# borgwang/tinynn-autograd

Hardware: NVIDIA B200
Metric: MLP train samples/sec (higher is better)
Workload: dtype f32 (tensor-core GEMMs: 3-term split on scaled fp16 hi/lo planes, fp32 accumulate)

## Files before the change

core/_backend.py:

```python
import ctypes
import gc
import os
import weakref

import numpy as np

_HERE = os.path.dirname(os.path.abspath(__file__))
_ROOT = os.path.dirname(_HERE)
LIB_PATH = os.environ.get(
    "TNN_B200_LIB", os.path.join(_ROOT, "tinynn-autograd_b200", "libtnn_b200.so"))

F32 = np.dtype(np.float32)
F64 = np.dtype(np.float64)
_DT_CODE = {F32: 0, F64: 1}
MAX_DIMS = 8

ADD, SUB, MUL, DIV, POW, MAXIMUM, MINIMUM, GE, GT, LE, LT, EQ = range(12)
MUL_GE, MUL_GT, MUL_LE, MUL_LT, MUL_EQ, DIV_BWD_B, POW_BWD_A, POW_BWD_B = range(20, 28)
NEG, EXP, LOG, COPY, CLIP, SCALE, CLIP_BWD, RECIP_MUL = range(40, 48)
RED_SUM, RED_MAX, RED_MIN = 0, 1, 2
OPT_SGD, OPT_ADAM, OPT_RMSPROP, OPT_MOMENTUM, OPT_ADAGRAD, OPT_ADADELTA = range(6)

_c_i64 = ctypes.c_int64
_c_i32 = ctypes.c_int32
_c_int = ctypes.c_int
_c_vp = ctypes.c_void_p
_c_dbl = ctypes.c_double
_c_sz = ctypes.c_size_t

_lib = None
_inited = False


class BackendError(RuntimeError):
    pass


_SIGNATURES = {
    "tnn_init": [_c_int],
    "tnn_shutdown": [],
    "tnn_sync": [],
    "tnn_device_info": [_c_vp, _c_vp, _c_vp, _c_vp, _c_vp],
    "tnn_device_count": [_c_vp],
    "tnn_alloc": [_c_sz, _c_vp],
    "tnn_free": [_c_vp],
    "tnn_pool_stats": [_c_vp, _c_vp, _c_vp],
    "tnn_pool_trim": [],
    "tnn_h2d": [_c_vp, _c_vp, _c_sz],
    "tnn_d2h": [_c_vp, _c_vp, _c_sz],
    "tnn_d2d": [_c_vp, _c_vp, _c_sz],
    "tnn_memset": [_c_vp, _c_int, _c_sz],
    "tnn_host_alloc": [_c_sz, _c_vp],
    "tnn_host_free": [_c_vp],
    "tnn_host_register": [_c_vp, _c_sz],
    "tnn_host_unregister": [_c_vp],
    "tnn_h2d_async_copy_stream": [_c_vp, _c_vp, _c_sz],
    "tnn_copy_stream_sync": [],
    "tnn_copy_wait_compute": [],
    "tnn_compute_wait_copy": [],
    "tnn_event_create": [_c_vp],
    "tnn_event_destroy": [_c_vp],
    "tnn_event_record": [_c_vp],
    "tnn_event_elapsed_ms": [_c_vp, _c_vp, _c_vp],
    "tnn_prof_enable": [_c_int],
    "tnn_prof_collect": [_c_vp, _c_vp],
    "tnn_l2_flush": [],
    "tnn_graph_begin": [],
    "tnn_graph_end": [_c_vp],
    "tnn_graph_abort": [],
    "tnn_graph_launch": [_c_vp],
    "tnn_graph_info": [_c_vp, _c_vp, _c_vp, _c_vp],
    "tnn_graph_destroy": [_c_vp],
    "tnn_ew": [_c_int, _c_int, _c_vp, _c_vp, _c_vp, _c_vp, _c_int, _c_vp, _c_vp, _c_vp, _c_vp,
               _c_dbl, _c_dbl, _c_int],
    "tnn_ew_flat": [_c_int, _c_int, _c_vp, _c_vp, _c_vp, _c_vp, _c_i64, _c_int, _c_dbl, _c_dbl,
                    _c_int],
    "tnn_cast": [_c_int, _c_vp, _c_int, _c_vp, _c_i64],
    "tnn_fill": [_c_int, _c_vp, _c_dbl, _c_i64],
    "tnn_reduce": [_c_int, _c_int, _c_vp, _c_vp, _c_i64, _c_i64, _c_i64],
    "tnn_unbroadcast": [_c_int, _c_vp, _c_vp, _c_int, _c_vp, _c_vp],
    "tnn_strided_copy": [_c_int, _c_vp, _c_vp, _c_int, _c_vp, _c_vp, _c_vp],
    "tnn_gather_rows": [_c_int, _c_vp, _c_vp, _c_vp, _c_i64, _c_i64, _c_i64],
    "tnn_scatter_rows": [_c_int, _c_vp, _c_vp, _c_vp, _c_i64, _c_i64, _c_i64],
    "tnn_gather_flat": [_c_int, _c_vp, _c_vp, _c_vp, _c_i64],
    "tnn_scatter_flat": [_c_int, _c_vp, _c_vp, _c_vp, _c_i64],
    "tnn_gemm_simt": [_c_int, _c_vp, _c_i64, _c_vp, _c_i64, _c_i64, _c_vp, _c_i64, _c_i64, _c_i64,
                      _c_i64, _c_i64, _c_vp, _c_int, _c_vp, _c_vp],
    "tnn_dense_bwd_simt": [_c_int, _c_vp, _c_vp, _c_vp, _c_vp, _c_vp, _c_vp, _c_vp, _c_int, _c_vp, _c_int,
                           _c_i64, _c_i64, _c_i64],
    "tnn_split_tf32": [_c_vp, _c_i64, _c_i64, _c_vp, _c_vp, _c_i64, _c_vp, _c_vp, _c_i64],
    "tnn_gemm_tf32x3": [_c_vp, _c_i64, _c_vp, _c_vp, _c_i64, _c_vp, _c_vp, _c_i64, _c_i64, _c_i64,
                        _c_i64, _c_vp, _c_int, _c_int, _c_vp, _c_vp, _c_vp, _c_i64, _c_vp],
    "tnn_split_tf32_bf16": [_c_vp, _c_i64, _c_i64, _c_vp, _c_vp, _c_vp, _c_i64],
    "tnn_gemm_tf32_bf16x2": [_c_vp, _c_i64, _c_vp, _c_vp, _c_vp, _c_i64, _c_vp, _c_vp, _c_vp, _c_i64,
                             _c_i64, _c_i64, _c_i64, _c_vp, _c_int, _c_int, _c_vp, _c_vp, _c_vp, _c_vp,
                             _c_i64, _c_vp],
    "tnn_f16_stats": [_c_vp, _c_i64, _c_vp, _c_int],
    "tnn_set_gemm_f16_cluster": [_c_int],
    "tnn_f16_meta_reset": [_c_vp],
    "tnn_split_f16": [_c_vp, _c_i64, _c_i64, _c_vp, _c_vp, _c_i64, _c_vp, _c_int],
    "tnn_gemm_f16x3": [_c_vp, _c_i64, _c_vp, _c_vp, _c_i64, _c_vp, _c_vp, _c_vp, _c_i64, _c_vp, _c_i64,
                       _c_i64, _c_i64, _c_vp, _c_int, _c_int, _c_vp, _c_vp, _c_vp],
    "tnn_split_tf32_bf16_cond": [_c_vp, _c_i64, _c_i64, _c_vp, _c_vp, _c_vp, _c_i64, _c_int,
                                 _c_vp, _c_i64, _c_i64, _c_vp, _c_vp, _c_vp, _c_i64, _c_int, _c_vp, _c_vp, _c_vp],
    "tnn_f16_stats_cond": [_c_vp, _c_i64, _c_vp, _c_int],
    "tnn_gemm_tf32_bf16x2_cond": [_c_vp, _c_i64, _c_vp, _c_vp, _c_vp, _c_i64, _c_vp, _c_vp, _c_vp, _c_i64,
                                  _c_i64, _c_i64, _c_i64, _c_vp, _c_int, _c_int, _c_vp, _c_vp, _c_vp, _c_vp],
    "tnn_set_gemm_cta_group": [_c_int],
    "tnn_set_gemm_ksplit": [_c_int],
    "tnn_set_gemm_group_m": [_c_int],
    "tnn_relu_fwd": [_c_int, _c_vp, _c_vp, _c_i64],
    "tnn_relu_bwd": [_c_int, _c_vp, _c_vp, _c_vp, _c_i64],
    "tnn_colsum": [_c_int, _c_vp, _c_vp, _c_i64, _c_i64],
    "tnn_ce_stats": [_c_int, _c_vp, _c_i64, _c_i64, _c_vp],
    "tnn_ce_merge_stats": [_c_int, _c_vp, _c_vp, _c_int],
    "tnn_ce_loss": [_c_int, _c_vp, _c_int, _c_vp, _c_i64, _c_i64, _c_vp, _c_dbl, _c_vp, _c_vp, _c_vp],
    "tnn_ce_fwd_small": [_c_int, _c_vp, _c_int, _c_vp, _c_i64, _c_i64, _c_dbl, _c_vp, _c_vp, _c_vp, _c_vp],
    "tnn_ce_bwd": [_c_int, _c_vp, _c_vp, _c_int, _c_vp, _c_i64, _c_i64, _c_vp, _c_vp, _c_dbl, _c_vp, _c_vp,
                   _c_vp],
    "tnn_set_gemm_reserved_sms": [_c_int],
    "tnn_d2h_async": [_c_vp, _c_vp, _c_sz, _c_vp],
    "tnn_event_sync": [_c_vp],
    "tnn_one_hot": [_c_int, _c_vp, _c_vp, _c_i64, _c_i64],
    "tnn_mlp_tail_workspace": [_c_int, _c_vp, _c_vp, _c_i64, _c_vp, _c_vp, _c_vp],
    "tnn_mlp_tail_step": [_c_int, _c_vp, _c_vp, _c_vp, _c_vp, _c_vp, _c_vp, _c_i64, _c_vp, _c_vp, _c_int,
                          _c_i64, _c_dbl, _c_vp, _c_vp, _c_vp, _c_vp, _c_vp, _c_vp, _c_vp],
    "tnn_opt_step": [_c_int, _c_int, _c_vp, _c_vp, _c_vp, _c_vp, _c_vp, _c_i64, _c_vp, _c_int],
    "tnn_opt_step_dev": [_c_int, _c_int, _c_vp, _c_vp, _c_vp, _c_vp, _c_vp, _c_i64, _c_vp],
    "tnn_nccl_unique_id": [_c_vp],
    "tnn_nccl_init": [_c_int, _c_int, _c_vp],
    "tnn_nccl_destroy": [],
    "tnn_allreduce_sum": [_c_int, _c_vp, _c_i64],
    "tnn_allgather": [_c_int, _c_vp, _c_vp, _c_i64],
    "tnn_comm_wait_compute": [],
    "tnn_compute_wait_comm": [],
    "tnn_allreduce_sum_comm": [_c_int, _c_vp, _c_i64],
    "tnn_nccl_version": [_c_vp],
}
EXPORTED_SYMBOLS = sorted(list(_SIGNATURES) + ["tnn_last_error", "tnn_stream", "tnn_launch_count",
                                                "tnn_alloc_ptr"])


def load_library():
    global _lib
    if _lib is not None:
        return _lib
    if not os.path.exists(LIB_PATH):
        raise BackendError(
            "libtnn_b200.so not found at %s -- build it with `python tinynn-autograd_b200/build.py` "
            "(there is no CPU fallback)" % LIB_PATH)
    lib = ctypes.CDLL(LIB_PATH)
    for name, argtypes in _SIGNATURES.items():
        fn = getattr(lib, name)
        fn.argtypes = argtypes
        fn.restype = _c_int
    lib.tnn_last_error.argtypes = []
    lib.tnn_last_error.restype = ctypes.c_char_p
    lib.tnn_stream.argtypes = []
    lib.tnn_stream.restype = _c_vp
    lib.tnn_launch_count.argtypes = []
    lib.tnn_launch_count.restype = ctypes.c_uint64
    lib.tnn_alloc_ptr.argtypes = [_c_sz]
    lib.tnn_alloc_ptr.restype = _c_vp
    _lib = lib
    return lib


def _raise(name):
    msg = _lib.tnn_last_error().decode("utf-8", "replace")
    raise BackendError("%s failed: %s" % (name, msg))


def init(device=None):
    global _inited
    if _inited:
        return
    lib = load_library()
    if device is None:
        device = int(os.environ.get("TNN_DEVICE", os.environ.get("LOCAL_RANK", "0")))
    if lib.tnn_init(int(device)):
        _raise("tnn_init")
    _inited = True


def is_initialized():
    return _inited


def sync():
    init()
    if _lib.tnn_sync():
        _raise("tnn_sync")


def launch_count():
    return int(_lib.tnn_launch_count()) if _lib is not None else 0


def device_info():
    init()
    sm, maj, mnr = _c_int(), _c_int(), _c_int()
    tot, l2 = _c_sz(), _c_sz()
    if _lib.tnn_device_info(ctypes.byref(sm), ctypes.byref(maj), ctypes.byref(mnr),
                            ctypes.byref(tot), ctypes.byref(l2)):
        _raise("tnn_device_info")
    return {"sm_count": sm.value, "cc": (maj.value, mnr.value), "total_mem": tot.value,
            "l2_bytes": l2.value}


def set_gemm_reserved_sms(n):
    init()
    if _lib.tnn_set_gemm_reserved_sms(int(n)):
        _raise("tnn_set_gemm_reserved_sms")


def pool_stats():
    a, b, c = _c_sz(), _c_sz(), _c_sz()
    _lib.tnn_pool_stats(ctypes.byref(a), ctypes.byref(b), ctypes.byref(c))
    return {"reserved": a.value, "in_use": b.value, "cuda_mallocs": c.value}


_SMALL_MAX = 1 << 20
_SMALL_KEEP = 64
_SMALL_CAP_BYTES = 256 << 20
_small_free = {}
_small_bytes = 0
_capturing = False


class _Buf(object):
    __slots__ = ("ptr", "nbytes", "klass", "__weakref__")

    def __init__(self, nbytes):
        self.nbytes = nbytes
        if nbytes <= _SMALL_MAX and not _capturing:
            klass = (nbytes + 511) & ~511
            lst = _small_free.get(klass)
            if lst:
                global _small_bytes
                _small_bytes -= klass
                self.ptr = lst.pop()
                self.klass = klass
                return
            nbytes = klass
            self.klass = klass
        else:
            self.klass = 0
        ptr = _lib.tnn_alloc_ptr(nbytes)
        if not ptr:
            self.ptr = None
            _raise("tnn_alloc")
        self.ptr = ptr

    def __del__(self):
        try:
            ptr = self.ptr
            if not ptr or _lib is None:
                return
            if self.klass and not _capturing:
                global _small_bytes
                lst = _small_free.setdefault(self.klass, [])
                if (len(lst) < (_SMALL_KEEP if self.klass <= 65536 else 8)
                        and _small_bytes + self.klass <= _SMALL_CAP_BYTES):
                    lst.append(ptr)
                    _small_bytes += self.klass
                    return
            _lib.tnn_free(ptr)
        except Exception:
            pass


def _prod(shape):
    n = 1
    for s in shape:
        n *= s
    return n


class DArray(object):
    __slots__ = ("buf", "ptr", "shape", "dtype", "size", "split", "aux", "__weakref__")

    def __init__(self, buf, ptr, shape, dtype):
        self.buf = buf
        self.ptr = ptr
        self.shape = shape
        self.dtype = dtype
        self.size = _prod(shape)
        self.split = None
        self.aux = None

    @property
    def ndim(self):
        return len(self.shape)

    @property
    def nbytes(self):
        return self.size * self.dtype.itemsize

    def view(self, shape, offset_elems=0):
        shape = tuple(int(s) for s in shape)
        return DArray(self.buf, self.ptr + offset_elems * self.dtype.itemsize, shape, self.dtype)

    def numpy(self):
        return to_numpy(self)

    def __array__(self, dtype=None, copy=None):
        a = to_numpy(self)
        return a if dtype is None else a.astype(dtype)

    def tolist(self):
        return to_numpy(self).tolist()

    def __repr__(self):
        return "DArray(shape=%s, dtype=%s)" % (self.shape, self.dtype.name)


class LazyReLU(DArray):
    __slots__ = ("_src", "_real")

    def __init__(self, src):
        self._src = src
        self._real = None
        self.shape = src.shape
        self.dtype = src.dtype
        self.size = src.size
        self.split = None
        self.aux = None

    def _materialise(self):
        if self._real is None:
            self._real = relu_fwd(self._src)
        return self._real

    @property
    def ptr(self):
        return self._materialise().ptr

    @property
    def buf(self):
        return self._materialise().buf


class LazyRows(DArray):
    __slots__ = ("_src", "_idx", "_real")

    def __init__(self, src, idx_window):
        self._src = src
        self._idx = idx_window
        self._real = None
        self.shape = (idx_window.size,) + tuple(src.shape[1:])
        self.dtype = src.dtype
        self.size = _prod(self.shape)
        self.split = None
        self.aux = None

    def gather_into(self, dst):
        assert dst.size == self.size and dst.dtype == self.dtype
        n = self.shape[0]
        row = _prod(self.shape[1:])
        if self.size and _lib.tnn_gather_rows(_DT_CODE[self.dtype], dst.ptr, self._src.ptr, self._idx.ptr, n,
                                              row, self._src.shape[0]):
            _raise("tnn_gather_rows")

    def _materialise(self):
        if self._real is None:
            self._real = gather_rows(self._src, self._idx, self.shape[0])
        return self._real

    @property
    def ptr(self):
        return self._materialise().ptr

    @property
    def buf(self):
        return self._materialise().buf

    def view(self, shape, offset_elems=0):
        return self._materialise().view(shape, offset_elems)


class LazyOneHot(DArray):
    __slots__ = ("_labels", "_dst", "_real")

    def __init__(self, labels, n_classes, dst):
        self._labels = labels
        self._dst = dst
        self._real = None
        self.shape = (labels.shape[0], int(n_classes))
        self.dtype = F32
        self.size = _prod(self.shape)
        self.split = None
        self.aux = None

    def _materialise(self):
        if self._real is None:
            one_hot_into(self._dst, self._labels.ptr, self.shape[0], self.shape[1])
            self._real = self._dst
        return self._real

    @property
    def labels_ptr(self):
        return self._labels.ptr

    @property
    def ptr(self):
        return self._materialise().ptr

    @property
    def buf(self):
        return self._materialise().buf

    def view(self, shape, offset_elems=0):
        return self._materialise().view(shape, offset_elems)


def device_dtype(np_dtype):
    dt = np.dtype(np_dtype)
    if dt == F32 or dt == np.float16:
        return F32
    if dt.kind in "fiub":
        return F64
    raise TypeError("unsupported dtype for a device tensor: %s" % dt)


def empty(shape, dtype):
    if not _inited:
        init()
    if type(shape) is not tuple:
        shape = tuple(int(s) for s in shape)
    if type(dtype) is not np.dtype:
        dtype = np.dtype(dtype)
    n = 1
    for s in shape:
        n *= s
    buf = _Buf((n if n > 0 else 1) * dtype.itemsize)
    return DArray(buf, buf.ptr, shape, dtype)


def from_numpy(arr, dtype=None):
    arr = np.asarray(arr)
    dt = device_dtype(arr.dtype if dtype is None else dtype)
    host = np.require(arr, dtype=dt, requirements="C")
    out = empty(host.shape, dt)
    if host.size:
        if _lib.tnn_h2d(out.ptr, host.ctypes.data, host.nbytes):
            _raise("tnn_h2d")
    return out


def upload_into(dst, host):
    host = np.require(host, dtype=dst.dtype, requirements="C")
    assert host.size == dst.size
    if host.size and _lib.tnn_h2d(dst.ptr, host.ctypes.data, host.nbytes):
        _raise("tnn_h2d")


def to_numpy(d):
    out = np.empty(d.shape, dtype=d.dtype)
    if d.size:
        if _lib.tnn_d2h(out.ctypes.data, d.ptr, out.nbytes):
            _raise("tnn_d2h")
    return out


def full(shape, value, dtype):
    out = empty(shape, dtype)
    if out.size:
        if _lib.tnn_fill(_DT_CODE[out.dtype], out.ptr, float(value), out.size):
            _raise("tnn_fill")
    return out


_ONES = {}


def ones_scalar(dtype):
    dtype = np.dtype(dtype)
    one = _ONES.get(dtype)
    if one is None:
        one = _ONES[dtype] = full((), 1.0, dtype)
    return one


def zeros(shape, dtype):
    out = empty(shape, dtype)
    if out.size:
        if _lib.tnn_memset(out.ptr, 0, out.nbytes):
            _raise("tnn_memset")
    return out


def memset_zero(d):
    if d.size and _lib.tnn_memset(d.ptr, 0, d.nbytes):
        _raise("tnn_memset")


def copy_into(dst, src):
    assert dst.size == src.size and dst.dtype == src.dtype
    if dst.size and _lib.tnn_d2d(dst.ptr, src.ptr, dst.nbytes):
        _raise("tnn_d2d")


def clone(d):
    out = empty(d.shape, d.dtype)
    copy_into(out, d)
    return out


def astype(d, dtype):
    dtype = np.dtype(dtype)
    if d.dtype == dtype:
        return d
    out = empty(d.shape, dtype)
    if d.size and _lib.tnn_cast(_DT_CODE[dtype], out.ptr, _DT_CODE[d.dtype], d.ptr, d.size):
        _raise("tnn_cast")
    return out


def upload_index(idx):
    idx = np.ascontiguousarray(idx, dtype=np.int64)
    out = empty(idx.shape, F64)
    if idx.size and _lib.tnn_h2d(out.ptr, idx.ctypes.data, idx.nbytes):
        _raise("tnn_h2d")
    return out


def _i64arr(vals):
    return (_c_i64 * len(vals))(*vals)


def _bstrides(shape, out_shape):
    nd = len(out_shape)
    pad = nd - len(shape)
    st = [0] * nd
    acc = 1
    for i in range(len(shape) - 1, -1, -1):
        if shape[i] != 1:
            st[pad + i] = acc
        acc *= shape[i]
    return st


def _common_dtype(*arrs):
    for a in arrs:
        if a.dtype == F64:
            return F64
    return F32


def ew(op, x, y=None, z=None, p0=0.0, p1=0.0, flags=0, out=None):
    ops_ = [a for a in (x, y, z) if a is not None]
    dt = _common_dtype(*ops_)
    ops_ = [a if a.dtype == dt else astype(a, dt) for a in ops_]
    if len(ops_) == 1:
        oshape = ops_[0].shape
    else:
        oshape = ops_[0].shape
        for a in ops_[1:]:
            if a.shape != oshape:
                oshape = np.broadcast_shapes(*[a.shape for a in ops_])
                break
    if out is None:
        out = empty(oshape, dt)
    n = out.size
    if n == 0:
        return out
    ptrs = [a.ptr for a in ops_] + [None] * (3 - len(ops_))
    mask = 0
    flat = True
    for i, a in enumerate(ops_):
        if a.size == 1:
            mask |= 1 << i
        elif a.shape != oshape:
            if a.size == n and _bstrides(a.shape, oshape) == _bstrides(oshape, oshape):
                continue
            flat = False
    if flat:
        if _lib.tnn_ew_flat(op, _DT_CODE[dt], out.ptr, ptrs[0], ptrs[1], ptrs[2], n, mask,
                            p0, p1, flags):
            _raise("tnn_ew_flat")
        return out
    nd = len(oshape)
    if nd > MAX_DIMS:
        raise ValueError("tensors of rank > %d are not supported" % MAX_DIMS)
    st = [_i64arr(_bstrides(a.shape, oshape)) for a in ops_] + [None] * (3 - len(ops_))
    if _lib.tnn_ew(op, _DT_CODE[dt], out.ptr, ptrs[0], ptrs[1], ptrs[2], nd, _i64arr(oshape),
                   st[0], st[1], st[2], p0, p1, flags):
        _raise("tnn_ew")
    return out


def add_inplace(dst, src):
    if src.dtype != dst.dtype:
        src = astype(src, dst.dtype)
    if _lib.tnn_ew_flat(ADD, _DT_CODE[dst.dtype], dst.ptr, dst.ptr, src.ptr, None, dst.size,
                        2 if (src.size == 1 and dst.size != 1) else 0, 0.0, 0.0, 0):
        _raise("tnn_ew_flat")
    return dst


def broadcast_to(d, shape):
    shape = tuple(shape)
    if d.shape == shape:
        return d
    out = empty(shape, d.dtype)
    oshape = np.broadcast_shapes(d.shape, shape)
    if tuple(oshape) != shape:
        raise ValueError("cannot broadcast %s to %s" % (d.shape, shape))
    if out.size:
        if _lib.tnn_ew(COPY, _DT_CODE[d.dtype], out.ptr, d.ptr, None, None, len(shape),
                       _i64arr(shape), _i64arr(_bstrides(d.shape, shape)), None, None, 0.0, 0.0, 0):
            _raise("tnn_ew")
    return out


def reduce(red_op, x, axis=None):
    if axis is None:
        outer, red, inner = 1, x.size, 1
        oshape = ()
    else:
        nd = x.ndim
        if not -nd <= axis < nd:
            raise np.exceptions.AxisError(axis, nd)
        axis %= nd
        outer = _prod(x.shape[:axis])
        red = x.shape[axis]
        inner = _prod(x.shape[axis + 1:])
        oshape = x.shape[:axis] + x.shape[axis + 1:]
    if red == 0 and red_op != RED_SUM:
        raise ValueError("zero-size array to reduction operation which has no identity")
    out = empty(oshape, x.dtype)
    if out.size:
        if _lib.tnn_reduce(red_op, _DT_CODE[x.dtype], out.ptr, x.ptr, outer, red, inner):
            _raise("tnn_reduce")
    return out


def unbroadcast(g, shape):
    shape = tuple(shape)
    if g.shape == shape:
        return g
    nd = g.ndim
    lead = nd - len(shape)
    if lead < 0:
        raise ValueError("gradient of rank %d for a tensor of rank %d" % (nd, len(shape)))
    keep = [0] * lead + [0 if s == 1 else 1 for s in shape]
    for i in range(len(shape)):
        if shape[i] != 1 and shape[i] != g.shape[lead + i]:
            raise ValueError("operands could not be broadcast together with shapes %s %s"
                             % (g.shape, shape))
    out = empty(shape, g.dtype)
    if out.size:
        if _lib.tnn_unbroadcast(_DT_CODE[g.dtype], out.ptr, g.ptr, nd, _i64arr(g.shape),
                                (_c_i32 * nd)(*keep)):
            _raise("tnn_unbroadcast")
    return out


def colsum(g, out=None):
    R, C = g.shape
    if out is None:
        out = empty((1, C), g.dtype)
    if _lib.tnn_colsum(_DT_CODE[g.dtype], out.ptr, g.ptr, R, C):
        _raise("tnn_colsum")
    return out


def _cstrides(shape):
    st = [0] * len(shape)
    acc = 1
    for i in range(len(shape) - 1, -1, -1):
        st[i] = acc
        acc *= shape[i]
    return st


def permute(x, axes):
    nd = x.ndim
    axes = [a % nd for a in axes]
    oshape = tuple(x.shape[a] for a in axes)
    out = empty(oshape, x.dtype)
    if out.size:
        xs = _cstrides(x.shape)
        if _lib.tnn_strided_copy(_DT_CODE[x.dtype], out.ptr, x.ptr, nd, _i64arr(oshape),
                                 _i64arr(_cstrides(oshape)), _i64arr([xs[a] for a in axes])):
            _raise("tnn_strided_copy")
    return out


def strided_copy(dst, dst_off, dst_strides, src, src_off, src_strides, shape):
    if _prod(shape) == 0:
        return
    isz = dst.dtype.itemsize
    if _lib.tnn_strided_copy(_DT_CODE[dst.dtype], dst.ptr + dst_off * isz, src.ptr + src_off * isz,
                             len(shape), _i64arr(shape), _i64arr(dst_strides), _i64arr(src_strides)):
        _raise("tnn_strided_copy")


def one_hot_into(out, labels_i32_ptr, n_rows, n_classes):
    if _lib.tnn_one_hot(_DT_CODE[out.dtype], out.ptr, labels_i32_ptr, n_rows, n_classes):
        _raise("tnn_one_hot")


def gather_rows(x, idx_dev, n_idx):
    row = _prod(x.shape[1:])
    out = empty((n_idx,) + x.shape[1:], x.dtype)
    if out.size and _lib.tnn_gather_rows(_DT_CODE[x.dtype], out.ptr, x.ptr, idx_dev.ptr, n_idx, row,
                                         x.shape[0]):
        _raise("tnn_gather_rows")
    return out


def scatter_rows(g, idx_dev, n_idx, shape):
    out = zeros(shape, g.dtype)
    row = _prod(shape[1:])
    if g.size and _lib.tnn_scatter_rows(_DT_CODE[g.dtype], out.ptr, g.ptr, idx_dev.ptr, n_idx, row,
                                        shape[0]):
        _raise("tnn_scatter_rows")
    return out


def gather_flat(x, idx_dev, oshape):
    out = empty(oshape, x.dtype)
    if out.size and _lib.tnn_gather_flat(_DT_CODE[x.dtype], out.ptr, x.ptr, idx_dev.ptr, out.size):
        _raise("tnn_gather_flat")
    return out


def scatter_flat(g, idx_dev, shape):
    out = zeros(shape, g.dtype)
    if g.size and _lib.tnn_scatter_flat(_DT_CODE[g.dtype], out.ptr, g.ptr, idx_dev.ptr, g.size):
        _raise("tnn_scatter_flat")
    return out


TC_MIN_MNK = int(os.environ.get("TNN_TC_MIN_MNK", str(1 << 29)))
TC_ENABLED = os.environ.get("TNN_TC", "1") != "0"
TC_MN_MAJOR = os.environ.get("TNN_TC_MN_MAJOR", "1") != "0"
TC_SPLIT = os.environ.get("TNN_GEMM_SPLIT", "f16")
LAZY_RELU_OUT = os.environ.get("TNN_LAZY_RELU", "1") != "0"
BF16_BYTES = 2
_split_epoch = 0


def new_split_epoch():
    global _split_epoch
    _split_epoch += 1


def _round4(n):
    return (n + 3) // 4 * 4


def _round8(n):
    return (n + 7) // 8 * 8


def _empty_16bit(rows, ld):
    return empty((rows, ld // 2), F32)


def split_planes_mix(x):
    cache = x.split
    if cache is None or cache.get("epoch") != _split_epoch:
        cache = {"epoch": _split_epoch}
        x.split = cache
    if "m" in cache:
        return cache["m"]
    R, C = x.shape
    ld = _round8(C)
    hi, h16, l16 = empty((R, ld), F32), _empty_16bit(R, ld), _empty_16bit(R, ld)
    if _lib.tnn_split_tf32_bf16(x.ptr, R, C, hi.ptr, h16.ptr, l16.ptr, ld):
        _raise("tnn_split_tf32_bf16")
    cache["m"] = (hi, h16, l16, ld)
    return cache["m"]


F16_PITCH_PAD = int(os.environ.get("TNN_F16_PITCH_PAD", "0"))


def _new_meta():
    return empty((8,), F32)


def split_planes_f16(x):
    cache = x.split
    if cache is None or cache.get("epoch") != _split_epoch:
        cache = {"epoch": _split_epoch}
        x.split = cache
    if "f" in cache:
        return cache["f"]
    R, C = x.shape
    ld = _round8(C) + F16_PITCH_PAD
    if type(x) is LazyReLU and x._real is None:
        src, relu_mode = x._src, 1
    else:
        src, relu_mode = x, 0
    meta = cache.get("stat")
    if meta is None:
        meta = _new_meta()
        if _lib.tnn_f16_stats(src.ptr, R * C, meta.ptr, relu_mode):
            _raise("tnn_f16_stats")
    elif _lib.tnn_f16_stats_cond(src.ptr, R * C, meta.ptr, relu_mode):
        _raise("tnn_f16_stats_cond")
    hf, l16 = _empty_16bit(R, ld), _empty_16bit(R, ld)
    if _lib.tnn_split_f16(src.ptr, R, C, hf.ptr, l16.ptr, ld, meta.ptr, relu_mode):
        _raise("tnn_split_f16")
    cache["f"] = (hf, l16, ld, meta, src if src is not x else None, relu_mode)
    return cache["f"]


_FALLBACK_PLANES = {}
_FALLBACK_CAP_BYTES = 16 << 30
_fallback_bytes = 0


def _fallback_planes(role, R, ld):
    if _capturing:
        return (empty((R, ld), F32), _empty_16bit(R, ld), _empty_16bit(R, ld))
    global _fallback_bytes
    key = (role, R, ld)
    p = _FALLBACK_PLANES.get(key)
    if p is None:
        if _fallback_bytes > _FALLBACK_CAP_BYTES:
            sync()
            _FALLBACK_PLANES.clear()
            _fallback_bytes = 0
        p = (empty((R, ld), F32), _empty_16bit(R, ld), _empty_16bit(R, ld))
        _FALLBACK_PLANES[key] = p
        _fallback_bytes += 8 * R * ld
    return p


def _matmul_f16(a, b, ta, tb, bias, out, flags, act, mask_src, M, N, K):
    a_hf, a_l16, lda, a_meta, a_src, a_relu = split_planes_f16(a)
    b_hf, b_l16, ldb, b_meta, b_src, b_relu = split_planes_f16(b)
    a_src = a if a_src is None else a_src
    b_src = b if b_src is None else b_src
    layout = (1 if ta else 0) | (0 if tb else 2)
    act_out = None
    stat = None
    if act:
        stat = _new_meta()
        if _lib.tnn_f16_meta_reset(stat.ptr):
            _raise("tnn_f16_meta_reset")
        if mask_src is None and LAZY_RELU_OUT:
            act_out = LazyReLU(out)
            flags |= 8
        else:
            act_out = empty((M, N), F32)
    real_act = act_out if (act and type(act_out) is not LazyReLU) else None
    bias_p = bias.ptr if bias is not None else None
    mask_p = mask_src.ptr if (act and mask_src is not None) else None
    if _lib.tnn_gemm_f16x3(out.ptr, N, a_hf.ptr, a_l16.ptr, lda, a_meta.ptr, b_hf.ptr, b_l16.ptr, ldb,
                           b_meta.ptr, M, N, K, bias_p, flags, layout,
                           real_act.ptr if real_act is not None else None, mask_p,
                           stat.ptr if stat is not None else None):
        _raise("tnn_gemm_f16x3")
    fa = _fallback_planes(0, a.shape[0], lda)
    fb = _fallback_planes(1, b.shape[0], ldb)
    if _lib.tnn_split_tf32_bf16_cond(a_src.ptr, a.shape[0], a.shape[1], fa[0].ptr, fa[1].ptr, fa[2].ptr, lda,
                                     a_relu, b_src.ptr, b.shape[0], b.shape[1], fb[0].ptr, fb[1].ptr,
                                     fb[2].ptr, ldb, b_relu, a_meta.ptr, b_meta.ptr,
                                     stat.ptr if stat is not None else None):
        _raise("tnn_split_tf32_bf16_cond")
    if _lib.tnn_gemm_tf32_bf16x2_cond(out.ptr, N, fa[0].ptr, fa[1].ptr, fa[2].ptr, lda, fb[0].ptr, fb[1].ptr,
                                      fb[2].ptr, ldb, M, N, K, bias_p, flags & 3, layout,
                                      real_act.ptr if real_act is not None else None, mask_p,
                                      a_meta.ptr, b_meta.ptr):
        _raise("tnn_gemm_tf32_bf16x2_cond")
    if act:
        act_out.split = {"epoch": _split_epoch, "stat": stat}
        return out, act_out
    return out


def split_planes(x, transposed, also_other=False):
    cache = x.split
    if cache is None or cache.get("epoch") != _split_epoch:
        cache = {"epoch": _split_epoch}
        x.split = cache
    key = "t" if transposed else "p"
    if key in cache:
        return cache[key]
    R, C = x.shape
    want_p = (not transposed) or (also_other and "p" not in cache)
    want_t = transposed or (also_other and "t" not in cache)
    hi = lo = hit = lot = None
    ldp = _round4(C)
    ldt = _round4(R)
    if want_p:
        hi, lo = empty((R, ldp), F32), empty((R, ldp), F32)
    if want_t:
        hit, lot = empty((C, ldt), F32), empty((C, ldt), F32)
    if _lib.tnn_split_tf32(x.ptr, R, C, hi.ptr if hi else None, lo.ptr if lo else None, ldp,
                           hit.ptr if hit else None, lot.ptr if lot else None, ldt):
        _raise("tnn_split_tf32")
    if want_p:
        cache["p"] = (hi, lo, ldp)
    if want_t:
        cache["t"] = (hit, lot, ldt)
    return cache[key]


def set_gemm_cta_group(cg):
    load_library()
    if _lib.tnn_set_gemm_cta_group(int(cg)):
        _raise("tnn_set_gemm_cta_group")


def set_gemm_f16_cluster(cl):
    load_library()
    if _lib.tnn_set_gemm_f16_cluster(int(cl)):
        _raise("tnn_set_gemm_f16_cluster")


def set_gemm_ksplit(ks):
    load_library()
    if _lib.tnn_set_gemm_ksplit(int(ks)):
        _raise("tnn_set_gemm_ksplit")


def use_tensor_cores(M, N, K, dtype):
    return (TC_ENABLED and dtype == F32 and M >= 64 and N >= 64 and K >= 32
            and M * N * K >= TC_MIN_MNK)


def matmul(a, b, ta=False, tb=False, bias=None, out=None, accumulate=False, relu=False,
           reuse_a=False, reuse_b=False, act=False, mask_src=None):
    if a.ndim != 2 or b.ndim != 2:
        raise ValueError("matmul: only 2-D operands are supported (got %s @ %s)" % (a.shape, b.shape))
    dt = _common_dtype(a, b)
    if a.dtype != dt:
        a = astype(a, dt)
    if b.dtype != dt:
        b = astype(b, dt)
    M, K = (a.shape[1], a.shape[0]) if ta else a.shape
    K2, N = (b.shape[1], b.shape[0]) if tb else b.shape
    if K != K2:
        raise ValueError("matmul: shapes %s and %s not aligned" % ((M, K), (K2, N)))
    if out is None:
        out = empty((M, N), dt)
        accumulate = False
    elif out.dtype != dt or out.shape != (M, N):
        raise ValueError("matmul: bad output array")
    if bias is not None and bias.dtype != dt:
        bias = astype(bias, dt)
    act_out = empty((M, N), dt) if act else None
    if M == 0 or N == 0:
        return (out, act_out) if act else out
    flags = (1 if accumulate else 0) | (2 if relu else 0)
    if K > 0 and use_tensor_cores(M, N, K, dt) and TC_SPLIT == "f16":
        return _matmul_f16(a, b, ta, tb, bias, out, flags, act, mask_src, M, N, K)
    if K > 0 and use_tensor_cores(M, N, K, dt) and TC_SPLIT == "mix":
        a_hi, a_h16, a_l16, lda = split_planes_mix(a)
        b_hi, b_h16, b_l16, ldb = split_planes_mix(b)
        layout = (1 if ta else 0) | (0 if tb else 2)
        act_hi = act_h16 = act_l16 = None
        ld_act = _round8(N)
        if act:
            act_hi = empty((M, ld_act), F32)
            act_h16, act_l16 = _empty_16bit(M, ld_act), _empty_16bit(M, ld_act)
            if LAZY_RELU_OUT and mask_src is None:
                act_out = LazyReLU(out)
        if _lib.tnn_gemm_tf32_bf16x2(out.ptr, N, a_hi.ptr, a_h16.ptr, a_l16.ptr, lda, b_hi.ptr,
                                     b_h16.ptr, b_l16.ptr, ldb, M, N, K,
                                     bias.ptr if bias is not None else None, flags, layout,
                                     act_out.ptr if (act and type(act_out) is not LazyReLU) else None,
                                     act_hi.ptr if act else None,
                                     act_h16.ptr if act else None, act_l16.ptr if act else None,
                                     ld_act, mask_src.ptr if (act and mask_src is not None) else None):
            _raise("tnn_gemm_tf32_bf16x2")
        if act:
            act_out.split = {"epoch": _split_epoch, "m": (act_hi, act_h16, act_l16, ld_act)}
            return out, act_out
        return out
    if K > 0 and use_tensor_cores(M, N, K, dt):
        if TC_MN_MAJOR:
            a_hi, a_lo, lda = split_planes(a, transposed=False)
            b_hi, b_lo, ldb = split_planes(b, transposed=False)
            layout = (1 if ta else 0) | (0 if tb else 2)
        else:
            a_hi, a_lo, lda = split_planes(a, transposed=ta, also_other=reuse_a)
            b_hi, b_lo, ldb = split_planes(b, transposed=not tb, also_other=reuse_b)
            layout = 0
        act_hi = act_lo = None
        ld_act = _round4(N)
        if act:
            act_hi, act_lo = empty((M, ld_act), F32), empty((M, ld_act), F32)
        if _lib.tnn_gemm_tf32x3(out.ptr, N, a_hi.ptr, a_lo.ptr, lda, b_hi.ptr, b_lo.ptr, ldb, M, N,
                                K, bias.ptr if bias is not None else None, flags, layout,
                                act_out.ptr if act else None, act_hi.ptr if act else None,
                                act_lo.ptr if act else None, ld_act,
                                mask_src.ptr if (act and mask_src is not None) else None):
            _raise("tnn_gemm_tf32x3")
        if act:
            act_out.split = {"epoch": _split_epoch, "p": (act_hi, act_lo, ld_act)}
            return out, act_out
        return out
    a_rs, a_cs = (1, a.shape[1]) if ta else (a.shape[1], 1)
    b_rs, b_cs = (1, b.shape[1]) if tb else (b.shape[1], 1)
    if mask_src is not None and mask_src.dtype != dt:
        mask_src = astype(mask_src, dt)
    if _lib.tnn_gemm_simt(_DT_CODE[dt], out.ptr, N, a.ptr, a_rs, a_cs, b.ptr, b_rs, b_cs, M, N, K,
                          bias.ptr if bias is not None else None, flags & 1,
                          act_out.ptr if act else None,
                          mask_src.ptr if (act and mask_src is not None) else None):
        _raise("tnn_gemm_simt")
    if relu:
        if _lib.tnn_relu_fwd(_DT_CODE[dt], out.ptr, out.ptr, out.size):
            _raise("tnn_relu_fwd")
    return (out, act_out) if act else out


GROUPED_BWD_MAX_TILES = 1024


def dense_bwd_grouped_ok(B, K, N, dtype):
    if use_tensor_cores(B, K, N, dtype) or use_tensor_cores(K, N, B, dtype):
        return False
    t = lambda m, n: ((m + 31) // 32) * ((n + 31) // 32)
    return t(K, N) + t(B, K) + t(1, N) <= GROUPED_BWD_MAX_TILES


def dense_bwd_grouped(g, x, w, mask_src, need_dx, dw_out, dw_acc, db_out, db_acc):
    B, N = g.shape
    K = w.shape[0]
    dx = empty((B, K), g.dtype) if need_dx else None
    masked = empty((B, K), g.dtype) if (need_dx and mask_src is not None) else None
    if _lib.tnn_dense_bwd_simt(_DT_CODE[g.dtype], g.ptr, x.ptr, w.ptr,
                               mask_src.ptr if masked is not None else None,
                               dx.ptr if dx is not None else None,
                               masked.ptr if masked is not None else None,
                               dw_out.ptr, 1 if dw_acc else 0, db_out.ptr, 1 if db_acc else 0, B, K, N):
        _raise("tnn_dense_bwd_simt")
    return dx, masked


def relu_fwd(x):
    out = empty(x.shape, x.dtype)
    if x.size and _lib.tnn_relu_fwd(_DT_CODE[x.dtype], out.ptr, x.ptr, x.size):
        _raise("tnn_relu_fwd")
    return out


def relu_bwd(g, x):
    if g.dtype != x.dtype:
        g = astype(g, x.dtype)
    out = empty(x.shape, x.dtype)
    if x.size and _lib.tnn_relu_bwd(_DT_CODE[x.dtype], out.ptr, g.ptr, x.ptr, x.size):
        _raise("tnn_relu_bwd")
    return out


def ce_stats(z):
    B, C = z.shape
    stats = empty((2,), z.dtype)
    if _lib.tnn_ce_stats(_DT_CODE[z.dtype], z.ptr, B, C, stats.ptr):
        _raise("tnn_ce_stats")
    return stats


def ce_merge_stats(stats_all, n_ranks):
    out = empty((2,), stats_all.dtype)
    if _lib.tnn_ce_merge_stats(_DT_CODE[stats_all.dtype], out.ptr, stats_all.ptr, n_ranks):
        _raise("tnn_ce_merge_stats")
    return out


def _ce_labels(y):
    if type(y) is LazyOneHot and y._real is None:
        return None, y.labels_ptr
    return y.ptr, None


def ce_loss(z, y, stats, m_global):
    B, C = z.shape
    q = empty((B,), z.dtype)
    loss = empty((), z.dtype)
    y_ptr, lab_ptr = _ce_labels(y)
    if _lib.tnn_ce_loss(_DT_CODE[z.dtype], z.ptr, _DT_CODE[y.dtype], y_ptr, B, C, stats.ptr,
                        float(m_global), q.ptr, loss.ptr, lab_ptr):
        _raise("tnn_ce_loss")
    return loss, q


def ce_small_ok(B, C):
    return B <= 2048 and B * C <= 16384


def ce_fwd_small(z, y, m_global, want_dz=False):
    B, C = z.shape
    stats, q, loss = empty((2,), z.dtype), empty((B,), z.dtype), empty((), z.dtype)
    dz = empty((B, C), z.dtype) if want_dz else None
    if _lib.tnn_ce_fwd_small(_DT_CODE[z.dtype], z.ptr, _DT_CODE[y.dtype], y.ptr, B, C,
                             float(m_global), stats.ptr, q.ptr, loss.ptr, dz.ptr if want_dz else None):
        _raise("tnn_ce_fwd_small")
    return stats, loss, q, dz


def is_ones_scalar(g):
    one = _ONES.get(np.dtype(g.dtype))
    return one is not None and g is one


def ce_bwd(z, y, stats, q, m_global, g):
    B, C = z.shape
    dz = empty((B, C), z.dtype)
    if g.dtype != z.dtype:
        g = astype(g, z.dtype)
    stat = None
    if z.dtype == F32 and TC_SPLIT == "f16" and TC_ENABLED and B * C >= (1 << 16):
        stat = _new_meta()
        if _lib.tnn_f16_meta_reset(stat.ptr):
            _raise("tnn_f16_meta_reset")
    y_ptr, lab_ptr = _ce_labels(y)
    if _lib.tnn_ce_bwd(_DT_CODE[z.dtype], dz.ptr, z.ptr, _DT_CODE[y.dtype], y_ptr, B, C, stats.ptr,
                       q.ptr, float(m_global), g.ptr, stat.ptr if stat is not None else None, lab_ptr):
        _raise("tnn_ce_bwd")
    if stat is not None:
        dz.split = {"epoch": _split_epoch, "stat": stat}
    return dz


class MLPTail(object):

    MAX_WIDTH = 256
    MAX_LAYERS = 6
    SMEM_LIMIT = 220 * 1024

    def __init__(self, dims, batch, n_grad):
        L = len(dims) - 1
        self.L, self.batch, self.n_grad = L, batch, n_grad
        self.in_dims = (_c_i64 * L)(*dims[:-1])
        self.out_dims = (_c_i64 * L)(*dims[1:])
        smem, n_ctas, scratch = _c_i64(), _c_i64(), _c_i64()
        if _lib.tnn_mlp_tail_workspace(L, self.in_dims, self.out_dims, batch, ctypes.byref(smem),
                                       ctypes.byref(n_ctas), ctypes.byref(scratch)):
            _raise("tnn_mlp_tail_workspace")
        self.smem_bytes, self.n_ctas = smem.value, n_ctas.value
        self.scratch = empty((scratch.value,), F32)
        self.stats = zeros((2 * self.n_ctas,), F32)
        self.loss_part = zeros((self.n_ctas,), F32)
        self.counters = zeros((16,), F32)
        self.logits = empty((batch, dims[-1]), F32)
        self.dlogits = self.scratch.view((batch, dims[-1]), scratch.value - batch * dims[-1])

    @classmethod
    def eligible(cls, dims, batch):
        init()
        L = len(dims) - 1
        if not (1 <= L <= cls.MAX_LAYERS) or any(d < 1 or d > cls.MAX_WIDTH for d in dims):
            return False
        if batch < 1 or batch > 256:
            return False
        floats = sum(dims[i] * (dims[i + 1] | 1) + (dims[i + 1] + 3) // 4 * 4 for i in range(L))
        floats = (floats + 3) // 4 * 4 + 12 * sum(dims) + 4 * 256
        return floats * 4 <= cls.SMEM_LIMIT

    def run(self, ws, bs, grad_base, grad_offsets, n_grad, z1, y, m_global, dz1, loss_out):
        if n_grad != self.n_grad:
            raise ValueError("MLPTail was laid out for %d gradient elements, got %d" % (self.n_grad, n_grad))
        wp = (_c_vp * self.L)(*[w.ptr for w in ws])
        bp = (_c_vp * self.L)(*[b.ptr for b in bs])
        go = (_c_i64 * (2 * self.L))(*grad_offsets)
        if _lib.tnn_mlp_tail_step(self.L, self.in_dims, self.out_dims, wp, bp, go, grad_base.ptr, n_grad,
                                  z1.ptr, y.ptr, _DT_CODE[y.dtype], self.batch, float(m_global), dz1.ptr,
                                  loss_out.ptr, self.scratch.ptr, self.stats.ptr, self.loss_part.ptr,
                                  self.counters.ptr, self.logits.ptr):
            _raise("tnn_mlp_tail_step")


def opt_step(opt, param, step_out, grad, s0, s1, hyper):
    n = grad.size
    if isinstance(hyper, DArray):
        if _lib.tnn_opt_step_dev(opt, _DT_CODE[grad.dtype], param.ptr if param is not None else None,
                                 step_out.ptr if step_out is not None else None, grad.ptr,
                                 s0.ptr if s0 is not None else None,
                                 s1.ptr if s1 is not None else None, n, hyper.ptr):
            _raise("tnn_opt_step_dev")
        return
    h = (_c_dbl * len(hyper))(*hyper)
    if _lib.tnn_opt_step(opt, _DT_CODE[grad.dtype], param.ptr if param is not None else None,
                         step_out.ptr if step_out is not None else None, grad.ptr,
                         s0.ptr if s0 is not None else None, s1.ptr if s1 is not None else None,
                         n, h, len(hyper)):
        _raise("tnn_opt_step")


class PinnedArray(object):

    def __init__(self, shape, dtype):
        init()
        self.shape = tuple(shape)
        self.dtype = np.dtype(dtype)
        nbytes = max(_prod(self.shape), 1) * self.dtype.itemsize
        p = _c_vp()
        if _lib.tnn_host_alloc(nbytes, ctypes.byref(p)):
            _raise("tnn_host_alloc")
        self.ptr = p.value
        self.nbytes = nbytes
        raw = (ctypes.c_char * nbytes).from_address(self.ptr)
        self.array = np.frombuffer(raw, dtype=self.dtype, count=_prod(self.shape)).reshape(self.shape)

    def __del__(self):
        try:
            if self.ptr and _lib is not None:
                self.array = None
                _lib.tnn_host_free(self.ptr)
                self.ptr = None
        except Exception:
            pass


class RegisteredHostArray(object):

    def __init__(self, array):
        init()
        if not (isinstance(array, np.ndarray) and array.flags["C_CONTIGUOUS"]):
            raise ValueError("only C-contiguous numpy arrays can be pinned in place")
        self.array = array
        self.ptr = array.ctypes.data
        if _lib.tnn_host_register(self.ptr, array.nbytes):
            _raise("tnn_host_register")

    def row_address(self, row):
        return self.ptr + row * self.array.strides[0]

    def __del__(self):
        try:
            if self.ptr and _lib is not None:
                _lib.tnn_host_unregister(self.ptr)
                self.ptr = None
        except Exception:
            pass


def h2d_prefetch(dst, pinned):
    if _lib.tnn_copy_wait_compute():
        _raise("tnn_copy_wait_compute")
    src = pinned if isinstance(pinned, int) else pinned.ptr
    if _lib.tnn_h2d_async_copy_stream(dst.ptr, src, dst.nbytes):
        _raise("tnn_h2d_async_copy_stream")


def copy_stream_sync():
    if _lib.tnn_copy_stream_sync():
        _raise("tnn_copy_stream_sync")


def wait_prefetch():
    if _lib.tnn_compute_wait_copy():
        _raise("tnn_compute_wait_copy")


_pinned_free = {}


class AsyncRead(object):

    def __init__(self, d):
        init()
        self.shape, self.dtype = d.shape, d.dtype
        nbytes = max(d.nbytes, 1)
        free = _pinned_free.get(nbytes)
        self.pin = free.pop() if free else PinnedArray((nbytes,), np.uint8)
        self.event = Event()
        self._src = d
        self._value = None
        if _lib.tnn_d2h_async(self.pin.ptr, d.ptr, d.nbytes, self.event.ptr):
            _raise("tnn_d2h_async")

    def result(self):
        if self._value is None:
            if _lib.tnn_event_sync(self.event.ptr):
                _raise("tnn_event_sync")
            n = int(np.prod(self.shape)) if self.shape else 1
            self._value = np.frombuffer(self.pin.array, dtype=self.dtype, count=n).reshape(self.shape).copy()
            _pinned_free.setdefault(self.pin.nbytes, []).append(self.pin)
            self.pin = self._src = None
        return self._value


class Event(object):
    def __init__(self):
        init()
        p = _c_vp()
        if _lib.tnn_event_create(ctypes.byref(p)):
            _raise("tnn_event_create")
        self.ptr = p.value

    def record(self):
        if _lib.tnn_event_record(self.ptr):
            _raise("tnn_event_record")

    def elapsed_ms_since(self, start):
        ms = ctypes.c_float()
        if _lib.tnn_event_elapsed_ms(start.ptr, self.ptr, ctypes.byref(ms)):
            _raise("tnn_event_elapsed_ms")
        return ms.value

    def __del__(self):
        try:
            if self.ptr and _lib is not None:
                _lib.tnn_event_destroy(self.ptr)
        except Exception:
            pass


_LIVE_GRAPHS = weakref.WeakSet()


def destroy_all_graphs():
    for g in list(_LIVE_GRAPHS):
        g.destroy()


class StepGraph(object):

    def __init__(self):
        init()
        self.handle = None
        _LIVE_GRAPHS.add(self)

    def capture(self):
        return _Capture(self)

    def replay(self):
        if not self.handle:
            raise BackendError("this recorded step was destroyed (process group torn down?)")
        if _lib.tnn_graph_launch(self.handle):
            _raise("tnn_graph_launch")

    def info(self):
        a, b, c = _c_sz(), _c_sz(), _c_sz()
        if _lib.tnn_graph_info(self.handle, ctypes.byref(a), ctypes.byref(b), ctypes.byref(c)):
            _raise("tnn_graph_info")
        return {"nodes": a.value, "kernel_nodes": b.value, "blocks": c.value}

    def destroy(self):
        if self.handle and _lib is not None:
            _lib.tnn_graph_destroy(self.handle)
        self.handle = None

    def __del__(self):
        try:
            self.destroy()
        except Exception:
            pass


class _Capture(object):
    def __init__(self, graph):
        self.graph = graph

    def __enter__(self):
        if self.graph.handle:
            raise BackendError("StepGraph already holds a captured step")
        global _capturing
        gc.collect()
        self._gc_was_enabled = gc.isenabled()
        gc.disable()
        if _lib.tnn_graph_begin():
            if self._gc_was_enabled:
                gc.enable()
            _raise("tnn_graph_begin")
        _capturing = True
        return self.graph

    def __exit__(self, exc_type, exc, tb):
        global _capturing
        _capturing = False
        try:
            if exc_type is not None:
                _lib.tnn_graph_abort()
                return False
            h = _c_vp()
            if _lib.tnn_graph_end(ctypes.byref(h)):
                _raise("tnn_graph_end")
            self.graph.handle = h.value
            return False
        finally:
            if self._gc_was_enabled:
                gc.enable()


def prof_enable(family):
    init()
    if _lib.tnn_prof_enable(family):
        _raise("tnn_prof_enable")


def prof_collect():
    ms, n = _c_dbl(), ctypes.c_uint64()
    if _lib.tnn_prof_collect(ctypes.byref(ms), ctypes.byref(n)):
        _raise("tnn_prof_collect")
    return ms.value, n.value


def l2_flush():
    init()
    if _lib.tnn_l2_flush():
        _raise("tnn_l2_flush")
```

include/tnn_b200.h:

```cpp
#ifndef TNN_B200_H
#define TNN_B200_H

#include <stddef.h>
#include <stdint.h>

#ifdef __cplusplus
extern "C" {
#endif

#define TNN_MAX_DIMS 8
#define TNN_F32 0
#define TNN_F64 1

enum {
  TNN_OP_ADD = 0,
  TNN_OP_SUB = 1,
  TNN_OP_MUL = 2,
  TNN_OP_DIV = 3,
  TNN_OP_POW = 4,
  TNN_OP_MAXIMUM = 5,
  TNN_OP_MINIMUM = 6,
  TNN_OP_GE = 7,
  TNN_OP_GT = 8,
  TNN_OP_LE = 9,
  TNN_OP_LT = 10,
  TNN_OP_EQ = 11,
  TNN_OP_MUL_GE = 20,
  TNN_OP_MUL_GT = 21,
  TNN_OP_MUL_LE = 22,
  TNN_OP_MUL_LT = 23,
  TNN_OP_MUL_EQ = 24,
  TNN_OP_DIV_BWD_B = 25,
  TNN_OP_POW_BWD_A = 26,
  TNN_OP_POW_BWD_B = 27,
  TNN_OP_NEG = 40,
  TNN_OP_EXP = 41,
  TNN_OP_LOG = 42,
  TNN_OP_COPY = 43,
  TNN_OP_CLIP = 44,
  TNN_OP_SCALE = 45,
  TNN_OP_CLIP_BWD = 46,
  TNN_OP_RECIP_MUL = 47
};

enum { TNN_RED_SUM = 0, TNN_RED_MAX = 1, TNN_RED_MIN = 2 };

enum {
  TNN_OPT_SGD = 0,
  TNN_OPT_ADAM = 1,
  TNN_OPT_RMSPROP = 2,
  TNN_OPT_MOMENTUM = 3,
  TNN_OPT_ADAGRAD = 4,
  TNN_OPT_ADADELTA = 5
};

const char* tnn_last_error(void);
int tnn_init(int device);
int tnn_shutdown(void);
int tnn_sync(void);
int tnn_device_info(int* sm_count, int* cc_major, int* cc_minor, size_t* total_mem, size_t* l2_bytes);
int tnn_device_count(int* n);
void* tnn_stream(void);
uint64_t tnn_launch_count(void);

int tnn_alloc(size_t nbytes, void** out);
void* tnn_alloc_ptr(size_t nbytes);
int tnn_free(void* p);
int tnn_pool_stats(size_t* reserved_bytes, size_t* in_use_bytes, size_t* n_cuda_malloc);
int tnn_pool_trim(void);
int tnn_h2d(void* dst, const void* src, size_t nbytes);
int tnn_d2h(void* dst, const void* src, size_t nbytes);
int tnn_d2h_async(void* pinned_dst, const void* src, size_t nbytes, void* done_event);
int tnn_event_sync(void* ev);
int tnn_d2d(void* dst, const void* src, size_t nbytes);
int tnn_memset(void* dst, int byte, size_t nbytes);
int tnn_host_alloc(size_t nbytes, void** out);
int tnn_host_free(void* p);
int tnn_host_register(void* p, size_t nbytes);
int tnn_host_unregister(void* p);
int tnn_h2d_async_copy_stream(void* dst, const void* pinned_src, size_t nbytes);
int tnn_copy_stream_sync(void);
int tnn_copy_wait_compute(void);
int tnn_compute_wait_copy(void);
int tnn_event_create(void** ev);
int tnn_event_destroy(void* ev);
int tnn_event_record(void* ev);
int tnn_event_elapsed_ms(void* start, void* stop, float* ms);
int tnn_prof_enable(int family);
int tnn_prof_collect(double* total_ms, uint64_t* n_launches);
int tnn_l2_flush(void);

int tnn_graph_begin(void);
int tnn_graph_end(void** graph_out);
int tnn_graph_abort(void);
int tnn_graph_launch(void* graph);
int tnn_graph_info(void* graph, size_t* n_nodes, size_t* n_kernel_nodes, size_t* n_blocks);
int tnn_graph_destroy(void* graph);

int tnn_ew(int op, int dtype, void* out, const void* x, const void* y, const void* z,
           int ndim, const int64_t* shape,
           const int64_t* xs, const int64_t* ys, const int64_t* zs,
           double p0, double p1, int flags);
int tnn_ew_flat(int op, int dtype, void* out, const void* x, const void* y, const void* z,
                int64_t n, int scalar_mask, double p0, double p1, int flags);
int tnn_cast(int dst_dtype, void* dst, int src_dtype, const void* src, int64_t n);
int tnn_fill(int dtype, void* dst, double value, int64_t n);

int tnn_reduce(int red_op, int dtype, void* out, const void* x,
               int64_t outer, int64_t red, int64_t inner);
int tnn_unbroadcast(int dtype, void* out, const void* grad, int ndim,
                    const int64_t* gshape, const int32_t* keep);

int tnn_strided_copy(int dtype, void* dst, const void* src, int ndim, const int64_t* shape,
                     const int64_t* dst_strides, const int64_t* src_strides);
int tnn_gather_rows(int dtype, void* out, const void* x, const int64_t* idx_dev,
                    int64_t n_idx, int64_t row_elems, int64_t n_rows_src);
int tnn_scatter_rows(int dtype, void* out, const void* g, const int64_t* idx_dev,
                     int64_t n_idx, int64_t row_elems, int64_t n_rows_dst);
int tnn_gather_flat(int dtype, void* out, const void* x, const int64_t* idx_dev, int64_t n);
int tnn_scatter_flat(int dtype, void* out, const void* g, const int64_t* idx_dev, int64_t n);
int tnn_one_hot(int dtype, void* out, const int32_t* labels_dev, int64_t B, int64_t C);

int tnn_gemm_simt(int dtype, void* C, int64_t ldc, const void* A, int64_t a_rs, int64_t a_cs,
                  const void* B, int64_t b_rs, int64_t b_cs, int64_t M, int64_t N, int64_t K,
                  const void* bias, int flags, void* act_out, const void* mask_src);
int tnn_dense_bwd_simt(int dtype, const void* g, const void* x, const void* w, const void* mask_src,
                       void* dx, void* dx_masked, void* dw, int dw_accumulate, void* db,
                       int db_accumulate, int64_t B, int64_t K, int64_t N);
int tnn_split_tf32(const float* x, int64_t R, int64_t C,
                   float* hi, float* lo, int64_t ldp, float* hiT, float* loT, int64_t ldt);
int tnn_gemm_tf32x3(float* D, int64_t ldd,
                    const float* a_hi, const float* a_lo, int64_t lda,
                    const float* b_hi, const float* b_lo, int64_t ldb,
                    int64_t M, int64_t N, int64_t K, const float* bias, int flags, int layout,
                    float* act_out, float* act_hi, float* act_lo, int64_t ld_act,
                    const float* mask_src);
int tnn_split_tf32_bf16(const float* x, int64_t R, int64_t C, float* hi, void* h16, void* l16,
                        int64_t ld);
int tnn_gemm_tf32_bf16x2(float* D, int64_t ldd,
                         const float* a_hi, const void* a_h16, const void* a_l16, int64_t lda,
                         const float* b_hi, const void* b_h16, const void* b_l16, int64_t ldb,
                         int64_t M, int64_t N, int64_t K, const float* bias, int flags, int layout,
                         float* act_out, float* act_hi, void* act_h16, void* act_l16, int64_t ld_act,
                         const float* mask_src);
int tnn_f16_stats(const float* x, int64_t n, void* meta, int relu_mode);
int tnn_set_gemm_f16_cluster(int cl);
int tnn_f16_meta_reset(void* meta);
int tnn_split_f16(const float* x, int64_t R, int64_t C, void* hf, void* l16, int64_t ld, void* meta,
                  int relu_mode);
int tnn_gemm_f16x3(float* D, int64_t ldd, const void* a_hf, const void* a_l16, int64_t lda,
                   const void* a_meta, const void* b_hf, const void* b_l16, int64_t ldb,
                   const void* b_meta, int64_t M, int64_t N, int64_t K, const float* bias, int flags,
                   int layout, float* act_out, const float* mask_src, void* stat_meta);
int tnn_split_tf32_bf16_cond(const float* xa, int64_t Ra, int64_t Ca, float* hia, void* h16a, void* l16a,
                             int64_t lda, int relu_a, const float* xb, int64_t Rb, int64_t Cb, float* hib,
                             void* h16b, void* l16b, int64_t ldb, int relu_b, const void* meta_a,
                             const void* meta_b, void* result_meta);
int tnn_f16_stats_cond(const float* x, int64_t n, void* meta, int relu_mode);
int tnn_gemm_tf32_bf16x2_cond(float* D, int64_t ldd, const float* a_hi, const void* a_h16,
                              const void* a_l16, int64_t lda, const float* b_hi, const void* b_h16,
                              const void* b_l16, int64_t ldb, int64_t M, int64_t N, int64_t K,
                              const float* bias, int flags, int layout, float* act_out,
                              const float* mask_src, const void* meta_a, const void* meta_b);
int tnn_set_gemm_cta_group(int cg);
int tnn_set_gemm_reserved_sms(int n);
int tnn_set_gemm_ksplit(int ks);
int tnn_set_gemm_group_m(int gm);

int tnn_relu_fwd(int dtype, void* out, const void* x, int64_t n);
int tnn_relu_bwd(int dtype, void* dx, const void* g, const void* x, int64_t n);
int tnn_colsum(int dtype, void* out, const void* g, int64_t R, int64_t C);

int tnn_ce_stats(int dtype, const void* z, int64_t B, int64_t C, void* stats_dev);
int tnn_ce_merge_stats(int dtype, void* stats_out_dev, const void* stats_all_dev, int n_ranks);
int tnn_ce_loss(int dtype, const void* z, int y_dtype, const void* y, int64_t B, int64_t C,
                const void* stats_dev, double m_global, void* q_dev, void* loss_dev,
                const int32_t* labels_dev);
int tnn_ce_fwd_small(int dtype, const void* z, int y_dtype, const void* y, int64_t B, int64_t C,
                     double m_global, void* stats_dev, void* q_dev, void* loss_dev,
                     void* dz_dev );
int tnn_ce_bwd(int dtype, void* dz, const void* z, int y_dtype, const void* y, int64_t B, int64_t C,
               const void* stats_dev, const void* q_dev, double m_global, const void* g_dev,
               void* stat_meta ,
               const int32_t* labels_dev);

int tnn_mlp_tail_workspace(int n_layers, const int64_t* in_dims, const int64_t* out_dims, int64_t batch,
                           int64_t* smem_bytes, int64_t* n_ctas, int64_t* scratch_floats);
int tnn_mlp_tail_step(int n_layers, const int64_t* in_dims, const int64_t* out_dims, const void* const* w,
                      const void* const* b, const int64_t* grad_off, void* grad, int64_t n_grad,
                      const void* z1, const void* y, int y_dtype, int64_t B, double m_global, void* dz1,
                      void* loss_out, void* scratch, void* stats, void* loss_part, void* counters,
                      void* logits_out );

int tnn_opt_step(int opt, int dtype, void* param, void* step_out, const void* grad, void* s0,
                 void* s1, int64_t n, const double* h, int n_h);
int tnn_opt_step_dev(int opt, int dtype, void* param, void* step_out, const void* grad, void* s0,
                     void* s1, int64_t n, const double* h_dev);

int tnn_nccl_unique_id(void* id128);
int tnn_nccl_init(int rank, int world, const void* id128);
int tnn_nccl_destroy(void);
int tnn_allreduce_sum(int dtype, void* buf, int64_t n);
int tnn_allgather(int dtype, void* recv, const void* send, int64_t n_per_rank);
int tnn_comm_wait_compute(void);
int tnn_compute_wait_comm(void);
int tnn_allreduce_sum_comm(int dtype, void* buf, int64_t n);
int tnn_nccl_version(int* v);

#ifdef __cplusplus
}
#endif
#endif
```

tinynn-autograd_b200/build.py:

```python
import concurrent.futures
import os
import shutil
import subprocess
import sys

HERE = os.path.dirname(os.path.abspath(__file__))
ROOT = os.path.dirname(HERE)
CSRC = os.path.join(HERE, "csrc")
OBJ = os.path.join(HERE, "build")
LIB = os.path.join(HERE, "libtnn_b200.so")

SOURCES = ["runtime.cu", "elementwise.cu", "reduce.cu", "layout.cu", "gemm_simt.cu",
           "gemm_tc.cu", "gemm_f16.cu", "fused.cu", "mlp_fused.cu", "comm.cu"]
HEADERS = [os.path.join(CSRC, "common.cuh"), os.path.join(CSRC, "math.cuh"), os.path.join(CSRC, "tc_ptx.cuh"),
           os.path.join(ROOT, "include", "tnn_b200.h")]

NVCC_FLAGS = ["-gencode", "arch=compute_100a,code=sm_100a", "-O3", "-lineinfo", "-std=c++17",
              "-Xcompiler", "-fPIC", "-diag-suppress", "550", "-split-compile", "0"]
NO_FMAD = {"elementwise.cu", "fused.cu", "reduce.cu"}


def _nvcc():
    return shutil.which("nvcc") or "/usr/local/cuda/bin/nvcc"


def _stale(target, deps):
    if not os.path.exists(target):
        return True
    t = os.path.getmtime(target)
    return any(os.path.getmtime(d) > t for d in deps)


def _compile(src, force):
    obj = os.path.join(OBJ, src.replace(".cu", ".o"))
    path = os.path.join(CSRC, src)
    if not force and not _stale(obj, [path] + HEADERS):
        return obj, False
    cmd = [_nvcc()] + NVCC_FLAGS + (["-fmad=false"] if src in NO_FMAD else []) + ["-c", path, "-o", obj]
    r = subprocess.run(cmd, capture_output=True, text=True)
    if r.returncode != 0:
        raise RuntimeError("nvcc failed for %s:\n%s\n%s" % (src, r.stdout[-4000:], r.stderr[-4000:]))
    return obj, True


def build(force=False, verbose=True):
    os.makedirs(OBJ, exist_ok=True)
    with concurrent.futures.ThreadPoolExecutor(max_workers=min(8, len(SOURCES))) as ex:
        results = list(ex.map(lambda s: _compile(s, force), SOURCES))
    objs = [o for o, _ in results]
    rebuilt = any(changed for _, changed in results)
    if rebuilt or _stale(LIB, objs):
        cmd = [_nvcc(), "-shared", "-o", LIB] + objs + ["-ldl"]
        r = subprocess.run(cmd, capture_output=True, text=True)
        if r.returncode != 0:
            raise RuntimeError("link failed:\n%s\n%s" % (r.stdout[-4000:], r.stderr[-4000:]))
        if verbose:
            print("built", LIB)
    elif verbose:
        print("up to date:", LIB)
    return LIB


if __name__ == "__main__":
    build(force="--force" in sys.argv)
```

tinynn-autograd_b200/csrc/fused.cu:

```cuda
#include <algorithm>

#include "common.cuh"
#include "math.cuh"

namespace tnn {

template <typename T>
struct V4 {
  static constexpr int W = sizeof(T) == 4 ? 4 : 2;
  using type = typename std::conditional<sizeof(T) == 4, float4, double2>::type;
  union U {
    type v;
    T e[W];
  };
};

static inline bool al16(const void* p) { return (reinterpret_cast<uintptr_t>(p) & 15) == 0; }

template <typename T, bool BWD, bool VEC>
__global__ void __launch_bounds__(256) relu_kernel(T* out, const T* g, const T* x, int64_t n) {
  constexpr int W = VEC ? V4<T>::W : 1;
  constexpr int U = 4;
  const int64_t nv = n / W;
  const int64_t stride = (int64_t)gridDim.x * blockDim.x;
  for (int64_t i0 = (int64_t)blockIdx.x * blockDim.x + threadIdx.x; i0 < nv; i0 += U * stride) {
    if constexpr (VEC) {
      typename V4<T>::U a[U], b[U], r;
#pragma unroll
      for (int u = 0; u < U; ++u) {
        const int64_t i = i0 + u * stride;
        if (i < nv) {
          a[u].v = reinterpret_cast<const typename V4<T>::type*>(x)[i];
          if (BWD) b[u].v = reinterpret_cast<const typename V4<T>::type*>(g)[i];
        }
      }
#pragma unroll
      for (int u = 0; u < U; ++u) {
        const int64_t i = i0 + u * stride;
        if (i < nv) {
#pragma unroll
          for (int k = 0; k < W; ++k)
            r.e[k] = BWD ? (a[u].e[k] >= T(0) ? b[u].e[k] : b[u].e[k] * T(0)) : m_max(a[u].e[k], T(0));
          reinterpret_cast<typename V4<T>::type*>(out)[i] = r.v;
        }
      }
    } else {
#pragma unroll
      for (int u = 0; u < U; ++u) {
        const int64_t i = i0 + u * stride;
        if (i < nv) {
          T a = x[i];
          out[i] = BWD ? (a >= T(0) ? g[i] : g[i] * T(0)) : m_max(a, T(0));
        }
      }
    }
  }
  if (VEC) {
    int64_t t = nv * W + (int64_t)blockIdx.x * blockDim.x + threadIdx.x;
    if (t < n) {
      T a = x[t];
      out[t] = BWD ? (a >= T(0) ? g[t] : g[t] * T(0)) : m_max(a, T(0));
    }
  }
}

template <typename T, bool BWD>
static int relu_launch(T* out, const T* g, const T* x, int64_t n) {
  if (n <= 0) return 0;
  bool vec = al16(out) && al16(x) && (!BWD || al16(g)) && n >= V4<T>::W;
  cudaStream_t st = ctx().stream;
  if (vec)
    relu_kernel<T, BWD, true><<<ew_grid(ceil_div(n, V4<T>::W), 256), 256, 0, st>>>(out, g, x, n);
  else
    relu_kernel<T, BWD, false><<<ew_grid(n, 256), 256, 0, st>>>(out, g, x, n);
  TNN_POST_LAUNCH();
  return 0;
}

template <typename T>
__device__ __forceinline__ T warp_sum(T v) {
#pragma unroll
  for (int o = 16; o > 0; o >>= 1) v += __shfl_xor_sync(0xffffffffu, v, o);
  return v;
}
template <typename T>
__device__ __forceinline__ T warp_max(T v) {
#pragma unroll
  for (int o = 16; o > 0; o >>= 1) v = m_max(v, __shfl_xor_sync(0xffffffffu, v, o));
  return v;
}
template <typename T, bool IS_MAX>
__device__ __forceinline__ T block_all_reduce(T v, T* sm ) {
  v = IS_MAX ? warp_max(v) : warp_sum(v);
  const int lane = threadIdx.x & 31, w = threadIdx.x >> 5;
  __syncthreads();
  if (lane == 0) sm[w] = v;
  __syncthreads();
  T r = sm[0];
#pragma unroll
  for (int i = 1; i < 8; ++i) r = IS_MAX ? m_max(r, sm[i]) : r + sm[i];
  return r;
}

template <typename T>
__global__ void __launch_bounds__(256) ce_stats_small_kernel(const T* z, int64_t n, T* stats) {
  __shared__ T sm[8];
  T mx = -INFINITY;
  for (int64_t i = threadIdx.x; i < n; i += 256) mx = m_max(mx, z[i]);
  mx = block_all_reduce<T, true>(mx, sm);
  T s = T(0);
  for (int64_t i = threadIdx.x; i < n; i += 256) s += m_exp(z[i] - mx);
  s = block_all_reduce<T, false>(s, sm);
  if (threadIdx.x == 0) {
    stats[0] = mx;
    stats[1] = s;
  }
}

template <typename T, bool VEC>
__global__ void __launch_bounds__(256)
ce_partial_max_kernel(const T* z, int64_t n, T* partial) {
  __shared__ T sm[8];
  constexpr int W = VEC ? V4<T>::W : 1;
  const int64_t nv = n / W;
  const int64_t stride = (int64_t)gridDim.x * blockDim.x;
  T mx = -INFINITY;
  for (int64_t i = (int64_t)blockIdx.x * blockDim.x + threadIdx.x; i < nv; i += stride) {
    if constexpr (VEC) {
      typename V4<T>::U a;
      a.v = reinterpret_cast<const typename V4<T>::type*>(z)[i];
#pragma unroll
      for (int k = 0; k < W; ++k) mx = m_max(mx, a.e[k]);
    } else {
      mx = m_max(mx, z[i]);
    }
  }
  if (VEC && blockIdx.x == 0) {
    int64_t t = nv * W + threadIdx.x;
    if (t < n) mx = m_max(mx, z[t]);
  }
  mx = block_all_reduce<T, true>(mx, sm);
  if (threadIdx.x == 0) partial[blockIdx.x] = mx;
}

template <typename T, bool VEC>
__global__ void __launch_bounds__(256)
ce_partial_sumexp_kernel(const T* z, int64_t n, const T* pmax, int n_pmax, T* psum, T* stats) {
  __shared__ T sm[8];
  T mx = -INFINITY;
  for (int i = threadIdx.x; i < n_pmax; i += 256) mx = m_max(mx, pmax[i]);
  mx = block_all_reduce<T, true>(mx, sm);
  constexpr int W = VEC ? V4<T>::W : 1;
  const int64_t nv = n / W;
  const int64_t stride = (int64_t)gridDim.x * blockDim.x;
  T s = T(0);
  if constexpr (VEC) {
    constexpr int U = 4;
    for (int64_t i0 = (int64_t)blockIdx.x * blockDim.x + threadIdx.x; i0 < nv; i0 += U * stride) {
      typename V4<T>::U a[U];
#pragma unroll
      for (int u = 0; u < U; ++u) {
        const int64_t i = i0 + u * stride;
        if (i < nv) a[u].v = reinterpret_cast<const typename V4<T>::type*>(z)[i];
      }
#pragma unroll
      for (int u = 0; u < U; ++u) {
        if (i0 + u * stride < nv) {
#pragma unroll
          for (int k = 0; k < W; ++k) s += m_exp(a[u].e[k] - mx);
        }
      }
    }
  } else {
    for (int64_t i = (int64_t)blockIdx.x * blockDim.x + threadIdx.x; i < nv; i += stride)
      s += m_exp(z[i] - mx);
  }
  if (VEC && blockIdx.x == 0) {
    int64_t t = nv * W + threadIdx.x;
    if (t < n) s += m_exp(z[t] - mx);
  }
  s = block_all_reduce<T, false>(s, sm);
  if (threadIdx.x == 0) {
    psum[blockIdx.x] = s;
    if (blockIdx.x == 0) stats[0] = mx;
  }
}

template <typename T>
__global__ void __launch_bounds__(256) ce_fold_sum_kernel(const T* psum, int n_psum, T* dst) {
  __shared__ T sm[8];
  T s = T(0);
  for (int i = threadIdx.x; i < n_psum; i += 256) s += psum[i];
  s = block_all_reduce<T, false>(s, sm);
  if (threadIdx.x == 0) dst[0] = s;
}

template <typename T>
__global__ void ce_merge_stats_kernel(T* out, const T* all, int n_ranks) {
  if (threadIdx.x == 0 && blockIdx.x == 0) {
    T mx = -INFINITY;
    for (int r = 0; r < n_ranks; ++r) mx = m_max(mx, all[2 * r]);
    T s = T(0);
    for (int r = 0; r < n_ranks; ++r) s += all[2 * r + 1] * m_exp(all[2 * r] - mx);
    out[0] = mx;
    out[1] = s;
  }
}

template <typename T, typename TY>
__global__ void __launch_bounds__(256)
ce_rows_kernel(const T* z, const TY* y, int64_t B, int64_t C, const T* stats, T* q, T* nll) {
  const T mx = stats[0], S = stats[1];
  const int lane = threadIdx.x & 31;
  const int64_t warps_total = (int64_t)gridDim.x * 8;
  for (int64_t r = (int64_t)blockIdx.x * 8 + (threadIdx.x >> 5); r < B; r += warps_total) {
    const T* zr = z + r * C;
    const TY* yr = y + r * C;
    T acc = T(0);
    for (int64_t j = lane; j < C; j += 32) {
      TY yy = yr[j];
      if (yy != TY(0)) acc += (m_exp(zr[j] - mx) / S) * (T)yy;
    }
    acc = warp_sum(acc);
    if (lane == 0) {
      q[r] = acc;
      nll[r] = -m_log(acc);
    }
  }
}

__global__ void __launch_bounds__(256)
ce_rows_vec_kernel(const float* z, const float* y, int64_t B, int64_t C, const float* stats, float* q,
                   float* nll) {
  const float mx = stats[0], S = stats[1];
  const int lane = threadIdx.x & 31;
  const int64_t warps_total = (int64_t)gridDim.x * 8;
  const int64_t nv = C / 4;
  for (int64_t r = (int64_t)blockIdx.x * 8 + (threadIdx.x >> 5); r < B; r += warps_total) {
    const float4* zr = reinterpret_cast<const float4*>(z + r * C);
    const float4* yr = reinterpret_cast<const float4*>(y + r * C);
    float acc = 0.f;
    for (int64_t j0 = lane; j0 < nv; j0 += 64) {
      const int64_t j1 = j0 + 32;
      const float4 ya = yr[j0], za = zr[j0];
      float4 yb = make_float4(0.f, 0.f, 0.f, 0.f), zb = yb;
      if (j1 < nv) {
        yb = yr[j1];
        zb = zr[j1];
      }
      if (ya.x != 0.f) acc += (m_exp(za.x - mx) / S) * ya.x;
      if (ya.y != 0.f) acc += (m_exp(za.y - mx) / S) * ya.y;
      if (ya.z != 0.f) acc += (m_exp(za.z - mx) / S) * ya.z;
      if (ya.w != 0.f) acc += (m_exp(za.w - mx) / S) * ya.w;
      if (yb.x != 0.f) acc += (m_exp(zb.x - mx) / S) * yb.x;
      if (yb.y != 0.f) acc += (m_exp(zb.y - mx) / S) * yb.y;
      if (yb.z != 0.f) acc += (m_exp(zb.z - mx) / S) * yb.z;
      if (yb.w != 0.f) acc += (m_exp(zb.w - mx) / S) * yb.w;
    }
    acc = warp_sum(acc);
    if (lane == 0) {
      q[r] = acc;
      nll[r] = -m_log(acc);
    }
  }
}

template <typename T>
__global__ void __launch_bounds__(256)
ce_rows_label_kernel(const T* z, const int32_t* labels, int64_t B, int64_t C, const T* stats, T* q, T* nll) {
  const T mx = stats[0], S = stats[1];
  const int64_t stride = (int64_t)gridDim.x * blockDim.x;
  for (int64_t r = (int64_t)blockIdx.x * blockDim.x + threadIdx.x; r < B; r += stride) {
    const int64_t l = labels[r];
    T acc = T(0);
    if (l >= 0 && l < C) acc += (m_exp(z[r * C + l] - mx) / S) * T(1);
    q[r] = acc;
    nll[r] = -m_log(acc);
  }
}

template <typename T>
__global__ void __launch_bounds__(256)
ce_fold_loss_kernel(const T* nll, int64_t B, T m, T* loss) {
  __shared__ T sm[8];
  T s = T(0);
  for (int64_t i = threadIdx.x; i < B; i += 256) s += nll[i];
  s = block_all_reduce<T, false>(s, sm);
  if (threadIdx.x == 0) loss[0] = s / m;
}

constexpr int CE_SMALL_MAX_ROWS = 2048;
template <typename T, bool IS_MAX>
__device__ __forceinline__ T block1024_reduce_first8(T v, T* sm ) {
  v = IS_MAX ? warp_max(v) : warp_sum(v);
  const int lane = threadIdx.x & 31, w = threadIdx.x >> 5;
  __syncthreads();
  if (lane == 0) sm[w] = v;
  __syncthreads();
  T r = sm[0];
#pragma unroll
  for (int i = 1; i < 8; ++i) r = IS_MAX ? m_max(r, sm[i]) : r + sm[i];
  return r;
}

constexpr int CE_SMALL_STAGE_BYTES = 16384;
template <typename T, typename TY>
__global__ void __launch_bounds__(1024)
ce_fwd_small_kernel(const T* z, const TY* y, int64_t B, int64_t C, T m, T* stats, T* q, T* loss, T* dz_out) {
  __shared__ T sm[32];
  __shared__ T nll[CE_SMALL_MAX_ROWS];
  constexpr int CE_SMALL_STAGE = CE_SMALL_STAGE_BYTES / (int)sizeof(T);
  __shared__ T zs[CE_SMALL_STAGE];
  const int64_t n = B * C;
  const bool first = threadIdx.x < 256;
  pdl_sync();
  const bool staged = n <= CE_SMALL_STAGE;
  if (staged) {
    for (int64_t i = threadIdx.x; i < n; i += 1024) zs[i] = z[i];
    __syncthreads();
  }
  const T* zz = staged ? zs : z;
  T mx = -INFINITY;
  if (first)
    for (int64_t i = threadIdx.x; i < n; i += 256) mx = m_max(mx, zz[i]);
  mx = block1024_reduce_first8<T, true>(mx, sm);
  T S = T(0);
  if (first)
    for (int64_t i = threadIdx.x; i < n; i += 256) S += m_exp(zz[i] - mx);
  S = block1024_reduce_first8<T, false>(S, sm);
  if (threadIdx.x == 0) {
    stats[0] = mx;
    stats[1] = S;
  }
  const int lane = threadIdx.x & 31, warp = threadIdx.x >> 5;
  constexpr int RU = 4;
  for (int64_t r0 = warp; r0 < B; r0 += 32 * RU) {
    T acc[RU];
#pragma unroll
    for (int u = 0; u < RU; ++u) {
      const int64_t r = r0 + 32 * u;
      acc[u] = T(0);
      if (r < B) {
        const T* zr = zz + r * C;
        const TY* yr = y + r * C;
        for (int64_t j = lane; j < C; j += 32) {
          TY yy = yr[j];
          if (yy != TY(0)) acc[u] += (m_exp(zr[j] - mx) / S) * (T)yy;
        }
      }
    }
#pragma unroll
    for (int u = 0; u < RU; ++u) {
      const int64_t r = r0 + 32 * u;
      const T a = warp_sum(acc[u]);
      if (lane == 0 && r < B) {
        q[r] = a;
        nll[r] = -m_log(a);
      }
    }
  }
  __syncthreads();
  T s = T(0);
  if (first)
    for (int64_t i = threadIdx.x; i < B; i += 256) s += nll[i];
  s = block1024_reduce_first8<T, false>(s, sm);
  if (threadIdx.x == 0) loss[0] = s / m;
  if (dz_out == nullptr) return;
  for (int64_t i = threadIdx.x; i < n; i += 1024) {
    const int64_t r = i / C;
    const T qm = q[r] * m;
    const T yv = (T)y[i];
    const T p = m_exp(zz[i] - mx) / S;
    T v = p;
    if (yv != T(0)) v = p - (yv * p) / qm;
    dz_out[i] = v;
  }
}

template <typename T, typename TY, bool VEC>
__global__ void __launch_bounds__(256)
ce_bwd_kernel(T* dz, const T* z, const TY* y, int64_t B, int64_t C, const T* stats, const T* q,
              T m, const T* gptr, unsigned int* absmax_out, const int32_t* labels) {
  constexpr int W = VEC ? 4 : 1;
  pdl_sync();
  const T mx = stats[0], S = stats[1], g = gptr[0];
  const int64_t nslot = C / W;
  unsigned int amax = 0u;
  for (int64_t r = blockIdx.y; r < B; r += gridDim.y) {
    const T qm = q[r] * m;
    const T* zr = z + r * C;
    const TY* yr = y + r * C;
    const int64_t lab = labels ? (int64_t)labels[r] : -1;
    T* dr = dz + r * C;
    for (int64_t c = (int64_t)blockIdx.x * 256 + threadIdx.x; c < nslot; c += (int64_t)gridDim.x * 256) {
      T zv[W], yv[W], out[W];
      if constexpr (VEC) {
        const float4 t = *reinterpret_cast<const float4*>(zr + c * 4);
        zv[0] = t.x; zv[1] = t.y; zv[2] = t.z; zv[3] = t.w;
        if (labels) {
#pragma unroll
          for (int k = 0; k < 4; ++k) yv[k] = (c * 4 + k == lab) ? T(1) : T(0);
        } else if constexpr (sizeof(TY) == 4) {
          const float4 u = *reinterpret_cast<const float4*>(yr + c * 4);
          yv[0] = u.x; yv[1] = u.y; yv[2] = u.z; yv[3] = u.w;
        } else {
          const double2 u0 = *reinterpret_cast<const double2*>(yr + c * 4);
          const double2 u1 = *reinterpret_cast<const double2*>(yr + c * 4 + 2);
          yv[0] = (T)u0.x; yv[1] = (T)u0.y; yv[2] = (T)u1.x; yv[3] = (T)u1.y;
        }
      } else {
        zv[0] = zr[c];
        yv[0] = labels ? ((c == lab) ? T(1) : T(0)) : (T)yr[c];
      }
#pragma unroll
      for (int k = 0; k < W; ++k) {
        T p = m_exp(zv[k] - mx) / S;
        T v = p;
        if (yv[k] != T(0)) v = p - (yv[k] * p) / qm;
        out[k] = g * v;
        if constexpr (sizeof(T) == 4) amax = max(amax, __float_as_uint((float)out[k]) & 0x7FFFFFFFu);
      }
      if constexpr (VEC) *reinterpret_cast<float4*>(dr + c * 4) = make_float4(out[0], out[1], out[2], out[3]);
      else dr[c] = out[0];
    }
  }
  if constexpr (sizeof(T) == 4) {
    if (absmax_out != nullptr) {
      amax = __reduce_max_sync(0xFFFFFFFFu, amax);
      if ((threadIdx.x & 31) == 0 && amax) atomicMax(absmax_out, amax);
    }
  }
}

struct OptH {
  double h[8];
};

template <int OPT, typename T>
__global__ void __launch_bounds__(256)
opt_kernel(T* param, T* step_out, const T* grad, T* s0, T* s1, int64_t n, OptH hh,
           const OptH* hdev) {
  pdl_sync();
  if (hdev) hh = *hdev;
  const int64_t stride = (int64_t)gridDim.x * blockDim.x;
  for (int64_t i = (int64_t)blockIdx.x * blockDim.x + threadIdx.x; i < n; i += stride) {
    const T g = grad[i];
    T step;
    if constexpr (OPT == TNN_OPT_SGD) {
      step = -(T)hh.h[0] * g;
    } else if constexpr (OPT == TNN_OPT_ADAM) {
      const T lr = (T)hh.h[0], omb1 = (T)(1.0 - hh.h[1]), omb2 = (T)(1.0 - hh.h[2]), eps = (T)hh.h[3];
      const T bc1 = (T)hh.h[4], bc2 = (T)hh.h[5];
      T m = s0[i], v = s1[i];
      m += omb1 * (g - m);
      v += omb2 * (g * g - v);
      s0[i] = m;
      s1[i] = v;
      T mh = m / bc1, vh = v / bc2;
      step = -lr * mh / (m_sqrt(vh) + eps);
    } else if constexpr (OPT == TNN_OPT_RMSPROP) {
      const T lr = (T)hh.h[0], omd = (T)(1.0 - hh.h[1]), mom_c = (T)hh.h[2], eps = (T)hh.h[3];
      T ms = s0[i], mom = s1[i];
      ms += omd * (g * g - ms);
      mom = mom_c * mom + lr * g / m_sqrt(ms + eps);
      s0[i] = ms;
      s1[i] = mom;
      step = -mom;
    } else if constexpr (OPT == TNN_OPT_MOMENTUM) {
      const T lr = (T)hh.h[0], mom_c = (T)hh.h[1];
      T acc = mom_c * s0[i] + g;
      s0[i] = acc;
      step = -lr * acc;
    } else if constexpr (OPT == TNN_OPT_ADAGRAD) {
      const T lr = (T)hh.h[0], eps = (T)hh.h[1];
      T G = s0[i] + g * g;
      s0[i] = G;
      step = -(lr / m_sqrt(G + eps)) * g;
    } else {
      const T lr = (T)hh.h[0], omd = (T)(1.0 - hh.h[1]), eps = (T)hh.h[2];
      T Eg = s0[i], delta = s1[i];
      Eg += omd * (g * g - Eg);
      T sd = m_sqrt(delta + eps);
      T d = g * (sd / m_sqrt(Eg + eps));
      step = -lr * d;
      delta += omd * (d * d - delta);
      s0[i] = Eg;
      s1[i] = delta;
    }
    if (param) {
      const T wd = (T)hh.h[7];
      const T p = param[i];
      if (wd != T(0)) step -= wd * p;
      param[i] = p + step;
    }
    if (step_out) step_out[i] = step;
  }
}

template <typename T>
__global__ void __launch_bounds__(256)
adam_vec_kernel(T* param, const T* grad, T* s0, T* s1, int64_t nv, OptH hh, const OptH* hdev) {
  pdl_sync();
  if (hdev) hh = *hdev;
  using VT = typename V4<T>::type;
  using U = typename V4<T>::U;
  constexpr int W = V4<T>::W;
  const T lr = (T)hh.h[0], omb1 = (T)(1.0 - hh.h[1]), omb2 = (T)(1.0 - hh.h[2]), eps = (T)hh.h[3];
  const T bc1 = (T)hh.h[4], bc2 = (T)hh.h[5];
  const T wd = (T)hh.h[7];
  const int64_t stride = (int64_t)gridDim.x * blockDim.x;
  for (int64_t i = (int64_t)blockIdx.x * blockDim.x + threadIdx.x; i < nv; i += stride) {
    U g, m, v, p;
    g.v = reinterpret_cast<const VT*>(grad)[i];
    m.v = reinterpret_cast<const VT*>(s0)[i];
    v.v = reinterpret_cast<const VT*>(s1)[i];
    p.v = reinterpret_cast<const VT*>(param)[i];
#pragma unroll
    for (int k = 0; k < W; ++k) {
      m.e[k] += omb1 * (g.e[k] - m.e[k]);
      v.e[k] += omb2 * (g.e[k] * g.e[k] - v.e[k]);
      T mh = m.e[k] / bc1, vh = v.e[k] / bc2;
      T step = -lr * mh / (m_sqrt(vh) + eps);
      if (wd != T(0)) step -= wd * p.e[k];
      p.e[k] += step;
    }
    reinterpret_cast<VT*>(s0)[i] = m.v;
    reinterpret_cast<VT*>(s1)[i] = v.v;
    reinterpret_cast<VT*>(param)[i] = p.v;
  }
}

template <typename T>
static int opt_dispatch(int opt, T* param, T* step_out, const T* grad, T* s0, T* s1, int64_t n,
                        const OptH& hh, const OptH* hdev) {
  cudaStream_t st = ctx().stream;
  int grid = ew_grid(n, 256);
  const bool pdl = grid <= 2 * ctx().sm_count;
  switch (opt) {
    case TNN_OPT_SGD:
      TNN_CUDA(launch_small(opt_kernel<TNN_OPT_SGD, T>, dim3(grid), dim3(256), st, pdl, 1u, param, step_out, grad, s0, s1, n, hh, hdev));
      break;
    case TNN_OPT_ADAM: {
      constexpr int W = V4<T>::W;
      if (param && !step_out && al16(param) && al16(grad) && al16(s0) && al16(s1) && n >= W) {
        int64_t nv = n / W;
        TNN_CUDA(launch_small(adam_vec_kernel<T>, dim3(ew_grid(nv, 256)), dim3(256), st, pdl, 1u, param, grad, s0, s1, nv, hh, hdev));
        ctx().launches++;
        int64_t done = nv * W;
        if (done < n)
          TNN_CUDA(launch_small(opt_kernel<TNN_OPT_ADAM, T>, dim3(1), dim3(256), st, pdl, 1u, param + done,
                                (T*)nullptr, grad + done, s0 + done, s1 + done, n - done, hh, hdev));
        else
          return 0;
      } else {
        TNN_CUDA(launch_small(opt_kernel<TNN_OPT_ADAM, T>, dim3(grid), dim3(256), st, pdl, 1u, param, step_out, grad, s0, s1, n, hh, hdev));
      }
      break;
    }
    case TNN_OPT_RMSPROP:
      TNN_CUDA(launch_small(opt_kernel<TNN_OPT_RMSPROP, T>, dim3(grid), dim3(256), st, pdl, 1u, param, step_out, grad, s0, s1, n, hh, hdev));
      break;
    case TNN_OPT_MOMENTUM:
      TNN_CUDA(launch_small(opt_kernel<TNN_OPT_MOMENTUM, T>, dim3(grid), dim3(256), st, pdl, 1u, param, step_out, grad, s0, s1, n, hh, hdev));
      break;
    case TNN_OPT_ADAGRAD:
      TNN_CUDA(launch_small(opt_kernel<TNN_OPT_ADAGRAD, T>, dim3(grid), dim3(256), st, pdl, 1u, param, step_out, grad, s0, s1, n, hh, hdev));
      break;
    case TNN_OPT_ADADELTA:
      TNN_CUDA(launch_small(opt_kernel<TNN_OPT_ADADELTA, T>, dim3(grid), dim3(256), st, pdl, 1u, param, step_out, grad, s0, s1, n, hh, hdev));
      break;
    default:
      TNN_FAIL("tnn_opt_step: unknown optimizer code");
  }
  TNN_POST_LAUNCH();
  return 0;
}

template <typename T>
static int ce_stats_impl(const T* z, int64_t B, int64_t C, T* stats) {
  const int64_t n = B * C;
  if (n <= 0) TNN_FAIL("tnn_ce_stats: empty logits");
  cudaStream_t st = ctx().stream;
  if (n <= 16384) {
    ce_stats_small_kernel<T><<<1, 256, 0, st>>>(z, n, stats);
    TNN_POST_LAUNCH();
    return 0;
  }
  const bool vec = al16(z);
  const int W = vec ? V4<T>::W : 1;
  int grid = ew_grid(ceil_div(n, W), 256, 4);
  void* scratch;
  if (get_scratch((size_t)grid * 2 * sizeof(T), &scratch)) return 1;
  T* pmax = (T*)scratch;
  T* psum = pmax + grid;
  if (vec) ce_partial_max_kernel<T, true><<<grid, 256, 0, st>>>(z, n, pmax);
  else ce_partial_max_kernel<T, false><<<grid, 256, 0, st>>>(z, n, pmax);
  TNN_POST_LAUNCH();
  if (vec) ce_partial_sumexp_kernel<T, true><<<grid, 256, 0, st>>>(z, n, pmax, grid, psum, stats);
  else ce_partial_sumexp_kernel<T, false><<<grid, 256, 0, st>>>(z, n, pmax, grid, psum, stats);
  TNN_POST_LAUNCH();
  ce_fold_sum_kernel<T><<<1, 256, 0, st>>>(psum, grid, stats + 1);
  TNN_POST_LAUNCH();
  return 0;
}

template <typename T, typename TY>
static int ce_loss_impl(const T* z, const TY* y, int64_t B, int64_t C, const T* stats, double m,
                        T* q, T* loss, const int32_t* labels) {
  cudaStream_t st = ctx().stream;
  void* scratch;
  if (get_scratch((size_t)B * sizeof(T), &scratch)) return 1;
  T* nll = (T*)scratch;
  if (labels) {
    ce_rows_label_kernel<T><<<ew_grid(B, 256), 256, 0, st>>>(z, labels, B, C, stats, q, nll);
    TNN_POST_LAUNCH();
    ce_fold_loss_kernel<T><<<1, 256, 0, st>>>(nll, B, (T)m, loss);
    TNN_POST_LAUNCH();
    return 0;
  }
  int grid = (int)std::min<int64_t>(ceil_div(B, 8), (int64_t)ctx().sm_count * 8);
  bool vec = false;
  if constexpr (sizeof(T) == 4 && sizeof(TY) == 4)
    vec = C >= 512 && C % 4 == 0 && al16(z) && al16(y);
  if (vec) {
    if constexpr (sizeof(T) == 4 && sizeof(TY) == 4)
      ce_rows_vec_kernel<<<grid, 256, 0, st>>>((const float*)z, (const float*)y, B, C, (const float*)stats,
                                               (float*)q, nll);
  } else {
    ce_rows_kernel<T, TY><<<grid, 256, 0, st>>>(z, y, B, C, stats, q, nll);
  }
  TNN_POST_LAUNCH();
  ce_fold_loss_kernel<T><<<1, 256, 0, st>>>(nll, B, (T)m, loss);
  TNN_POST_LAUNCH();
  return 0;
}

template <typename T, typename TY>
static int ce_bwd_impl(T* dz, const T* z, const TY* y, int64_t B, int64_t C, const T* stats,
                       const T* q, double m, const T* g, unsigned int* absmax_out, const int32_t* labels) {
  cudaStream_t st = ctx().stream;
  const bool vec = sizeof(T) == 4 && (C % 4 == 0) && al16(dz) && al16(z) && (labels || al16(y));
  const int64_t nslot = vec ? C / 4 : C;
  int gx = (int)std::min<int64_t>(ceil_div(nslot, 256), 64);
  int64_t gy = std::min<int64_t>(B, std::max<int64_t>(1, (int64_t)ctx().sm_count * 8 / gx));
  if (gy > 65535) gy = 65535;
  const bool pdl = (int64_t)gx * gy <= 2 * (int64_t)ctx().sm_count;
  if (vec) {
    if constexpr (sizeof(T) == 4)
      TNN_CUDA(launch_small(ce_bwd_kernel<T, TY, true>, dim3(gx, (unsigned)gy), dim3(256), st, pdl, 1u,
                            dz, z, y, B, C, stats, q, (T)m, g, absmax_out, labels));
  } else {
    TNN_CUDA(launch_small(ce_bwd_kernel<T, TY, false>, dim3(gx, (unsigned)gy), dim3(256), st, pdl, 1u,
                          dz, z, y, B, C, stats, q, (T)m, g, absmax_out, labels));
  }
  ctx().launches++;
  return 0;
}

}

using namespace tnn;

extern "C" {

int tnn_relu_fwd(int dtype, void* out, const void* x, int64_t n) {
  TNN_REQUIRE_INIT();
  if (dtype == TNN_F32) return relu_launch<float, false>((float*)out, nullptr, (const float*)x, n);
  if (dtype == TNN_F64) return relu_launch<double, false>((double*)out, nullptr, (const double*)x, n);
  TNN_FAIL("tnn_relu_fwd: bad dtype");
}

int tnn_relu_bwd(int dtype, void* dx, const void* g, const void* x, int64_t n) {
  TNN_REQUIRE_INIT();
  if (dtype == TNN_F32) return relu_launch<float, true>((float*)dx, (const float*)g, (const float*)x, n);
  if (dtype == TNN_F64) return relu_launch<double, true>((double*)dx, (const double*)g, (const double*)x, n);
  TNN_FAIL("tnn_relu_bwd: bad dtype");
}

int tnn_ce_stats(int dtype, const void* z, int64_t B, int64_t C, void* stats_dev) {
  TNN_REQUIRE_INIT();
  if (dtype == TNN_F32) return ce_stats_impl<float>((const float*)z, B, C, (float*)stats_dev);
  if (dtype == TNN_F64) return ce_stats_impl<double>((const double*)z, B, C, (double*)stats_dev);
  TNN_FAIL("tnn_ce_stats: bad dtype");
}

int tnn_ce_merge_stats(int dtype, void* stats_out_dev, const void* stats_all_dev, int n_ranks) {
  TNN_REQUIRE_INIT();
  cudaStream_t st = ctx().stream;
  if (dtype == TNN_F32)
    ce_merge_stats_kernel<float><<<1, 32, 0, st>>>((float*)stats_out_dev, (const float*)stats_all_dev, n_ranks);
  else if (dtype == TNN_F64)
    ce_merge_stats_kernel<double><<<1, 32, 0, st>>>((double*)stats_out_dev, (const double*)stats_all_dev, n_ranks);
  else
    TNN_FAIL("tnn_ce_merge_stats: bad dtype");
  TNN_POST_LAUNCH();
  return 0;
}

int tnn_ce_loss(int dtype, const void* z, int y_dtype, const void* y, int64_t B, int64_t C,
                const void* stats_dev, double m_global, void* q_dev, void* loss_dev,
                const int32_t* labels_dev) {
  TNN_REQUIRE_INIT();
  if (B <= 0 || C <= 0) TNN_FAIL("tnn_ce_loss: empty logits");
  if (!y && !labels_dev) TNN_FAIL("tnn_ce_loss: neither dense labels nor class indices");
  const int32_t* lab = labels_dev;
  if (dtype == TNN_F32 && y_dtype == TNN_F32)
    return ce_loss_impl<float, float>((const float*)z, (const float*)y, B, C, (const float*)stats_dev, m_global, (float*)q_dev, (float*)loss_dev, lab);
  if (dtype == TNN_F32 && y_dtype == TNN_F64)
    return ce_loss_impl<float, double>((const float*)z, (const double*)y, B, C, (const float*)stats_dev, m_global, (float*)q_dev, (float*)loss_dev, lab);
  if (dtype == TNN_F64 && y_dtype == TNN_F64)
    return ce_loss_impl<double, double>((const double*)z, (const double*)y, B, C, (const double*)stats_dev, m_global, (double*)q_dev, (double*)loss_dev, lab);
  if (dtype == TNN_F64 && y_dtype == TNN_F32)
    return ce_loss_impl<double, float>((const double*)z, (const float*)y, B, C, (const double*)stats_dev, m_global, (double*)q_dev, (double*)loss_dev, lab);
  TNN_FAIL("tnn_ce_loss: bad dtype");
}

int tnn_ce_fwd_small(int dtype, const void* z, int y_dtype, const void* y, int64_t B, int64_t C,
                     double m_global, void* stats_dev, void* q_dev, void* loss_dev, void* dz_dev) {
  TNN_REQUIRE_INIT();
  if (B <= 0 || C <= 0) TNN_FAIL("tnn_ce_fwd_small: empty logits");
  if (B > CE_SMALL_MAX_ROWS || B * C > 16384) TNN_FAIL("tnn_ce_fwd_small: at most 2048 rows and 16384 logits");
  cudaStream_t st = ctx().stream;
  if (dtype == TNN_F32 && y_dtype == TNN_F32)
    TNN_CUDA(launch_small(ce_fwd_small_kernel<float, float>, dim3(1), dim3(1024), st, true, 1u, (const float*)z, (const float*)y, B, C, (float)m_global, (float*)stats_dev, (float*)q_dev, (float*)loss_dev, (float*)dz_dev));
  else if (dtype == TNN_F32 && y_dtype == TNN_F64)
    TNN_CUDA(launch_small(ce_fwd_small_kernel<float, double>, dim3(1), dim3(1024), st, true, 1u, (const float*)z, (const double*)y, B, C, (float)m_global, (float*)stats_dev, (float*)q_dev, (float*)loss_dev, (float*)dz_dev));
  else if (dtype == TNN_F64 && y_dtype == TNN_F64)
    TNN_CUDA(launch_small(ce_fwd_small_kernel<double, double>, dim3(1), dim3(1024), st, true, 1u, (const double*)z, (const double*)y, B, C, m_global, (double*)stats_dev, (double*)q_dev, (double*)loss_dev, (double*)dz_dev));
  else if (dtype == TNN_F64 && y_dtype == TNN_F32)
    TNN_CUDA(launch_small(ce_fwd_small_kernel<double, float>, dim3(1), dim3(1024), st, true, 1u, (const double*)z, (const float*)y, B, C, m_global, (double*)stats_dev, (double*)q_dev, (double*)loss_dev, (double*)dz_dev));
  else
    TNN_FAIL("tnn_ce_fwd_small: bad dtype");
  TNN_POST_LAUNCH();
  return 0;
}

int tnn_ce_bwd(int dtype, void* dz, const void* z, int y_dtype, const void* y, int64_t B, int64_t C,
               const void* stats_dev, const void* q_dev, double m_global, const void* g_dev,
               void* stat_meta, const int32_t* labels_dev) {
  TNN_REQUIRE_INIT();
  if (B <= 0 || C <= 0) return 0;
  if (!y && !labels_dev) TNN_FAIL("tnn_ce_bwd: neither dense labels nor class indices");
  const int32_t* lab = labels_dev;
  unsigned int* am = (unsigned int*)stat_meta;
  if (am && dtype != TNN_F32) TNN_FAIL("tnn_ce_bwd: operand statistics are float32 only");
  if (dtype == TNN_F32 && y_dtype == TNN_F32)
    return ce_bwd_impl<float, float>((float*)dz, (const float*)z, (const float*)y, B, C, (const float*)stats_dev, (const float*)q_dev, m_global, (const float*)g_dev, am, lab);
  if (dtype == TNN_F32 && y_dtype == TNN_F64)
    return ce_bwd_impl<float, double>((float*)dz, (const float*)z, (const double*)y, B, C, (const float*)stats_dev, (const float*)q_dev, m_global, (const float*)g_dev, am, lab);
  if (dtype == TNN_F64 && y_dtype == TNN_F64)
    return ce_bwd_impl<double, double>((double*)dz, (const double*)z, (const double*)y, B, C, (const double*)stats_dev, (const double*)q_dev, m_global, (const double*)g_dev, am, lab);
  if (dtype == TNN_F64 && y_dtype == TNN_F32)
    return ce_bwd_impl<double, float>((double*)dz, (const double*)z, (const float*)y, B, C, (const double*)stats_dev, (const double*)q_dev, m_global, (const double*)g_dev, am, lab);
  TNN_FAIL("tnn_ce_bwd: bad dtype");
}

int tnn_opt_step(int opt, int dtype, void* param, void* step_out, const void* grad, void* s0,
                 void* s1, int64_t n, const double* h, int n_h) {
  TNN_REQUIRE_INIT();
  if (n <= 0) return 0;
  if (n_h < 0 || n_h > 8) TNN_FAIL("tnn_opt_step: at most 8 hyper-parameters");
  OptH hh;
  for (int i = 0; i < 8; ++i) hh.h[i] = i < n_h ? h[i] : 0.0;
  if (dtype == TNN_F32)
    return opt_dispatch<float>(opt, (float*)param, (float*)step_out, (const float*)grad, (float*)s0, (float*)s1, n, hh, nullptr);
  if (dtype == TNN_F64)
    return opt_dispatch<double>(opt, (double*)param, (double*)step_out, (const double*)grad, (double*)s0, (double*)s1, n, hh, nullptr);
  TNN_FAIL("tnn_opt_step: bad dtype");
}

int tnn_opt_step_dev(int opt, int dtype, void* param, void* step_out, const void* grad, void* s0,
                     void* s1, int64_t n, const double* h_dev) {
  TNN_REQUIRE_INIT();
  if (n <= 0) return 0;
  if (!h_dev) TNN_FAIL("tnn_opt_step_dev: h_dev is NULL");
  OptH hh = {};
  const OptH* hd = reinterpret_cast<const OptH*>(h_dev);
  if (dtype == TNN_F32)
    return opt_dispatch<float>(opt, (float*)param, (float*)step_out, (const float*)grad, (float*)s0, (float*)s1, n, hh, hd);
  if (dtype == TNN_F64)
    return opt_dispatch<double>(opt, (double*)param, (double*)step_out, (const double*)grad, (double*)s0, (double*)s1, n, hh, hd);
  TNN_FAIL("tnn_opt_step_dev: bad dtype");
}

}
```

tinynn-autograd_b200/csrc/gemm_f16.cu:

```cuda
#include <cuda.h>
#include <cuda_bf16.h>
#include <cuda_fp16.h>
#include <cudaTypedefs.h>

#include <algorithm>
#include <cstdlib>

#include "common.cuh"
#include "tc_ptx.cuh"

namespace tnn {
namespace tc {
extern int g_reserved_sms;
}
namespace f16 {

using namespace tnn::tc;

#ifndef TNN_F16_BK
#define TNN_F16_BK 64
#endif
#ifndef TNN_F16_STAGES
#define TNN_F16_STAGES (192 / TNN_F16_BK)
#endif
constexpr int BK = TNN_F16_BK;
constexpr int ROWS = 128;
constexpr int UMMA_N = 256;
constexpr int TILE_M = 256;
constexpr int UMMA_K = 16;
constexpr int PLANE_BYTES = ROWS * BK * 2;
constexpr int STAGE_BYTES = 4 * PLANE_BYTES;
constexpr int STAGES = TNN_F16_STAGES;
constexpr int CHUNK_KB = 256 / BK;
#ifndef TNN_F16_THREADS
#define TNN_F16_THREADS 384
#endif
constexpr int NUM_THREADS = TNN_F16_THREADS;
constexpr int EPI_WARP0 = NUM_THREADS == 320 ? 2 : 4;
constexpr uint32_t TMEM_COLS = 512;
constexpr int EPI_PATCH_BYTES = 8 * 4096;
constexpr int SMEM_BYTES = STAGES * STAGE_BYTES + 1024 + 256 + EPI_PATCH_BYTES;
#ifndef TNN_F16_KBOX_ROWS
#define TNN_F16_KBOX_ROWS 128
#endif
constexpr int KBOX_ROWS = TNN_F16_KBOX_ROWS;
constexpr int MN_BOX_BYTES = 64 * BK * 2;
constexpr float SMALL_LIMIT = 0.03125f;
constexpr unsigned int GUARD_FRACTION = 256;

struct Meta {
  unsigned int absmax;
  unsigned int need_stats;
  int exp;
  int safe;
  unsigned int n_small;
  unsigned int n_nz;
  unsigned int ticket;
  unsigned int pad;
};

__device__ __forceinline__ void meta_scale(unsigned int amax_bits, int& e, int& ok) {
  e = 0;
  ok = 1;
  if (amax_bits == 0u) return;
  if (amax_bits >= 0x7F800000u) { ok = 0; return; }
  const int ex = (int)(amax_bits >> 23) - 127;
  if (ex < -112) { ok = 0; return; }
  e = 14 - ex;
}

__device__ __forceinline__ float pow2f(int e) {
  return __int_as_float((e + 127) << 23);
}

template <bool MN>
__device__ __forceinline__ uint64_t make_desc(uint32_t saddr) {
  uint64_t d = 0;
  d |= (uint64_t)((saddr & 0x3FFFFu) >> 4);
  d |= (uint64_t)(MN ? (MN_BOX_BYTES >> 4) : 1) << 16;
  d |= (uint64_t)(((MN || BK == 64) ? 1024 : 512) >> 4) << 32;
  d |= (uint64_t)1 << 46;
  d |= (uint64_t)((MN || BK == 64) ? 2 : 4) << 61;
  return d;
}
__host__ __device__ constexpr uint32_t make_idesc(int a_fmt, int b_fmt, bool a_mn, bool b_mn) {
  return (1u << 4) | ((uint32_t)a_fmt << 7) | ((uint32_t)b_fmt << 10) | ((a_mn ? 1u : 0u) << 15) |
         ((b_mn ? 1u : 0u) << 16) | ((uint32_t)(UMMA_N >> 3) << 17) | ((uint32_t)(TILE_M >> 4) << 24);
}

__device__ __forceinline__ void tile_coords(int t, int tiles_m, int tiles_n, int group_m, int& tm, int& tn) {
  if (group_m == 1) {
    tm = t / tiles_n;
    tn = t - tm * tiles_n;
  } else if (group_m < 0) {
    const int gn = -group_m;
    const int per_panel = tiles_m * gn;
    const int g = t / per_panel;
    const int first_n = g * gn;
    const int cols = min(gn, tiles_n - first_n);
    const int r = t - g * per_panel;
    tm = r / cols;
    tn = first_n + r % cols;
  } else {
    const int per_group = group_m * tiles_n;
    const int g = t / per_group;
    const int first_m = g * group_m;
    const int rows = min(group_m, tiles_m - first_m);
    const int r = t - g * per_group;
    tm = first_m + r % rows;
    tn = r / rows;
  }
}

template <int CB>
__device__ __forceinline__ void patch_write(const float (&sum)[128], float4* patch, int lane, float f1,
                                            float f2, const float* bias_u, int colb, int N) {
#pragma unroll
  for (int c4 = 0; c4 < 8; ++c4) {
    float4 v = make_float4(sum[CB * 32 + c4 * 4] * f1 * f2, sum[CB * 32 + c4 * 4 + 1] * f1 * f2,
                           sum[CB * 32 + c4 * 4 + 2] * f1 * f2, sum[CB * 32 + c4 * 4 + 3] * f1 * f2);
    if (bias_u) {
      const int c = colb + c4 * 4;
      if (c + 3 < N) {
        const float4 b = *reinterpret_cast<const float4*>(bias_u + c);
        v.x += b.x; v.y += b.y; v.z += b.z; v.w += b.w;
      } else {
        if (c < N) v.x += bias_u[c];
        if (c + 1 < N) v.y += bias_u[c + 1];
        if (c + 2 < N) v.z += bias_u[c + 2];
      }
    }
    patch[lane * 8 + (c4 ^ (lane & 7))] = v;
  }
}

template <bool A_MN, bool B_MN, int CL>
__global__ void __launch_bounds__(NUM_THREADS, 1)
gemm_f16x3_kernel(const __grid_constant__ CUtensorMap map_a_h, const __grid_constant__ CUtensorMap map_a_l,
                  const __grid_constant__ CUtensorMap map_b_h, const __grid_constant__ CUtensorMap map_b_l,
                  float* __restrict__ D, int64_t ldd, int M, int N, int K,
                  const float* __restrict__ bias, int flags, int t_full, int tail_split,
                  unsigned int* __restrict__ tile_flags, float* __restrict__ act_out,
                  const float* __restrict__ mask_src, const Meta* __restrict__ meta_a,
                  const Meta* __restrict__ meta_b, Meta* __restrict__ stat_out, int group_m) {
  if (!(meta_a->safe && meta_b->safe)) return;
  extern __shared__ uint8_t smem_raw[];
  const uint32_t smem_base = (smem_u32(smem_raw) + 1023u) & ~1023u;
  uint8_t* smem_gen = smem_raw + (smem_base - smem_u32(smem_raw));
  const uint32_t bar_base = smem_base + STAGES * STAGE_BYTES;
  auto full_bar = [&](int s) { return bar_base + 8u * s; };
  auto empty_bar = [&](int s) { return bar_base + 8u * (STAGES + s); };
  auto tfull_bar = [&](int a) { return bar_base + 8u * (2 * STAGES + a); };
  auto tempty_bar = [&](int a) { return bar_base + 8u * (2 * STAGES + 2 + a); };
  const uint32_t tmem_ptr_smem = bar_base + 8u * (2 * STAGES + 4);
  volatile uint32_t* tmem_ptr_gen =
      reinterpret_cast<volatile uint32_t*>(smem_gen + STAGES * STAGE_BYTES + 8 * (2 * STAGES + 4));

  const int warp = threadIdx.x >> 5, lane = threadIdx.x & 31;
  const uint32_t cl_rank = cluster_ctarank();
  const uint32_t pair = cl_rank >> 1;
  const uint32_t cta_rank = cl_rank & 1u;
  const bool leader = cta_rank == 0;
  const uint16_t pair_mask = (uint16_t)(3u << (2 * pair));

  if (warp == 0 && lane == 0) {
    tma_prefetch_desc(&map_a_h);
    tma_prefetch_desc(&map_a_l);
    tma_prefetch_desc(&map_b_h);
    tma_prefetch_desc(&map_b_l);
    for (int s = 0; s < STAGES; ++s) {
      mbar_init(full_bar(s), 1);
      mbar_init(empty_bar(s), CL / 2);
    }
    for (int a = 0; a < 2; ++a) {
      mbar_init(tfull_bar(a), 1);
      mbar_init(tempty_bar(a), 16);
    }
    fence_barrier_init();
  }
  if (warp == 1) {
    tmem_alloc<2>(tmem_ptr_smem, TMEM_COLS);
    tmem_relinquish<2>();
  }
  tc_fence_before();
  cluster_sync_all();
  tc_fence_after();
  const uint32_t tmem_base = *tmem_ptr_gen;

  const int tiles_m = (M + TILE_M - 1) / TILE_M;
  const int tiles_n = (N + UMMA_N - 1) / UMMA_N;
  const int tiles_ns = CL == 4 ? (tiles_n + 1) / 2 : tiles_n;
  const int num_tiles = tiles_m * tiles_ns;
  const int num_kb = (K + BK - 1) / BK;
  const int group = blockIdx.x / CL;
  const int num_groups = gridDim.x / CL;
  const int tail_rem = num_tiles - t_full;
  const int num_units = t_full + tail_rem * tail_split;
  const int kb_per_split = (num_kb + tail_split - 1) / tail_split;
  auto decode = [&](int u, int& t, int& sp, int& kb_begin, int& kb_end) {
    if (u < t_full) {
      t = u; sp = 0; kb_begin = 0; kb_end = num_kb;
    } else {
      const int j = u - t_full;
      t = t_full + j % tail_rem;
      sp = j / tail_rem;
      kb_begin = sp * kb_per_split;
      kb_end = min(num_kb, kb_begin + kb_per_split);
    }
  };

  if (warp == 0) {
    if constexpr (NUM_THREADS == 384) asm volatile("setmaxnreg.dec.sync.aligned.u32 40;");
    if (lane == 0) {
      int stage = 0;
      uint32_t phase = 0;
      for (int u = group; u < num_units; u += num_groups) {
        int t, sp, kb_begin, kb_end;
        decode(u, t, sp, kb_begin, kb_end);
        int tm, tn;
        tile_coords((flags & 32) ? num_tiles - 1 - t : t, tiles_m, tiles_ns, group_m, tm, tn);
        if constexpr (CL == 4) tn = 2 * tn + (int)pair;
        const int row_a = tm * TILE_M + (int)cta_rank * ROWS;
        const int row_b = tn * UMMA_N + (int)cta_rank * ROWS;
        for (int kb = kb_begin; kb < kb_end; ++kb) {
          mbar_wait(empty_bar(stage), phase ^ 1u);
          const uint32_t sa_h = smem_base + stage * STAGE_BYTES;
          const uint32_t sa_l = sa_h + PLANE_BYTES;
          const uint32_t sb_h = sa_h + 2 * PLANE_BYTES;
          const uint32_t sb_l = sa_h + 3 * PLANE_BYTES;
          if (leader) mbar_expect_tx(full_bar(stage), (uint32_t)STAGE_BYTES * 2u);
          const int k0 = kb * BK;
          if (flags & 128) {
            if (leader)
              asm volatile("mbarrier.complete_tx.shared::cta.b64 [%0], %1;" ::"r"(full_bar(stage)), "r"((uint32_t)STAGE_BYTES * 2u) : "memory");
            if (++stage == STAGES) { stage = 0; phase ^= 1u; }
            continue;
          }
#ifdef TNN_F16_PREFETCH
          if (kb + TNN_F16_PREFETCH < kb_end) {
            const int kp = (kb + TNN_F16_PREFETCH) * BK;
            if constexpr (A_MN) {
#pragma unroll
              for (int j = 0; j < ROWS / 64; ++j) {
                tma_prefetch_l2_2d(&map_a_l, row_a + 64 * j, kp);
                tma_prefetch_l2_2d(&map_a_h, row_a + 64 * j, kp);
              }
            } else {
              tma_prefetch_l2_2d(&map_a_l, kp, row_a);
              tma_prefetch_l2_2d(&map_a_h, kp, row_a);
            }
            if constexpr (B_MN) {
#pragma unroll
              for (int j = 0; j < ROWS / 64; ++j) {
                tma_prefetch_l2_2d(&map_b_h, row_b + 64 * j, kp);
                tma_prefetch_l2_2d(&map_b_l, row_b + 64 * j, kp);
              }
            } else {
              tma_prefetch_l2_2d(&map_b_h, kp, row_b);
              tma_prefetch_l2_2d(&map_b_l, kp, row_b);
            }
          }
#endif
          if constexpr (CL == 4) {
            const uint16_t mc = (uint16_t)((1u << cta_rank) | (1u << (cta_rank + 2)));
            const uint32_t off = pair * (uint32_t)(PLANE_BYTES / 2);
            const int ra = row_a + 64 * (int)pair;
            if constexpr (A_MN) {
              tma_load_2d_pair_mc(sa_l + off, &map_a_l, full_bar(stage), ra, k0, mc);
              tma_load_2d_pair_mc(sa_h + off, &map_a_h, full_bar(stage), ra, k0, mc);
            } else {
              tma_load_2d_pair_mc(sa_l + off, &map_a_l, full_bar(stage), k0, ra, mc);
              tma_load_2d_pair_mc(sa_h + off, &map_a_h, full_bar(stage), k0, ra, mc);
            }
          } else if constexpr (A_MN) {
#pragma unroll
            for (int j = 0; j < ROWS / 64; ++j) {
              tma_load_2d<2>(sa_l + j * MN_BOX_BYTES, &map_a_l, full_bar(stage), row_a + 64 * j, k0);
              tma_load_2d<2>(sa_h + j * MN_BOX_BYTES, &map_a_h, full_bar(stage), row_a + 64 * j, k0);
            }
          } else {
#pragma unroll
            for (int j = 0; j < ROWS / KBOX_ROWS; ++j) {
              tma_load_2d<2>(sa_l + j * KBOX_ROWS * 128, &map_a_l, full_bar(stage), k0, row_a + j * KBOX_ROWS);
              tma_load_2d<2>(sa_h + j * KBOX_ROWS * 128, &map_a_h, full_bar(stage), k0, row_a + j * KBOX_ROWS);
            }
          }
          if constexpr (B_MN) {
#pragma unroll
            for (int j = 0; j < ROWS / 64; ++j) {
              tma_load_2d<2>(sb_h + j * MN_BOX_BYTES, &map_b_h, full_bar(stage), row_b + 64 * j, k0);
              tma_load_2d<2>(sb_l + j * MN_BOX_BYTES, &map_b_l, full_bar(stage), row_b + 64 * j, k0);
            }
          } else {
#pragma unroll
            for (int j = 0; j < ROWS / KBOX_ROWS; ++j) {
              tma_load_2d<2>(sb_h + j * KBOX_ROWS * 128, &map_b_h, full_bar(stage), k0, row_b + j * KBOX_ROWS);
              tma_load_2d<2>(sb_l + j * KBOX_ROWS * 128, &map_b_l, full_bar(stage), k0, row_b + j * KBOX_ROWS);
            }
          }
          if (++stage == STAGES) {
            stage = 0;
            phase ^= 1u;
          }
        }
      }
    }
  } else if (warp == 1) {
    if constexpr (NUM_THREADS == 384) asm volatile("setmaxnreg.dec.sync.aligned.u32 40;");
    if (leader && lane == 0) {
      constexpr uint32_t idesc = make_idesc(0, 0, A_MN, B_MN);
      int stage = 0;
      uint32_t phase = 0;
      int acc = 0;
      uint32_t acc_phase = 0;
#ifdef TNN_F16_PROBE
      long long w_full = 0, w_empty = 0, t_begin = clock64();
#endif
      for (int u = group; u < num_units; u += num_groups) {
        int t, sp, kb_begin, kb_end;
        decode(u, t, sp, kb_begin, kb_end);
        for (int kb0 = kb_begin; kb0 < kb_end; kb0 += CHUNK_KB) {
#ifdef TNN_F16_PROBE
          long long p0 = clock64();
#endif
          mbar_wait(tempty_bar(acc), acc_phase ^ 1u);
#ifdef TNN_F16_PROBE
          w_empty += clock64() - p0;
#endif
          tc_fence_after();
          const uint32_t tmem_d = tmem_base + (uint32_t)(acc * UMMA_N);
          const int kb1 = min(kb0 + CHUNK_KB, kb_end);
          for (int kb = kb0; kb < kb1; ++kb) {
#ifdef TNN_F16_PROBE
            long long p1 = clock64();
#endif
            mbar_wait(full_bar(stage), phase);
#ifdef TNN_F16_PROBE
            w_full += clock64() - p1;
#endif
            tc_fence_after();
            const uint32_t sa_h = smem_base + stage * STAGE_BYTES;
            const uint32_t sa_l = sa_h + PLANE_BYTES;
            const uint32_t sb_h = sa_h + 2 * PLANE_BYTES;
            const uint32_t sb_l = sa_h + 3 * PLANE_BYTES;
            if (!(flags & 256))
#pragma unroll
            for (int k = 0; k < BK / UMMA_K; ++k) {
              const uint32_t koff_a = (uint32_t)(k * (A_MN ? 2048 : 32));
              const uint32_t koff_b = (uint32_t)(k * (B_MN ? 2048 : 32));
              const uint64_t da_h = make_desc<A_MN>(sa_h + koff_a);
              const uint64_t da_l = make_desc<A_MN>(sa_l + koff_a);
              const uint64_t db_h = make_desc<B_MN>(sb_h + koff_b);
              const uint64_t db_l = make_desc<B_MN>(sb_l + koff_b);
              umma_bf16<2>(tmem_d, da_l, db_h, idesc, (kb != kb0 || k != 0) ? 1u : 0u);
              umma_bf16<2>(tmem_d, da_h, db_l, idesc, 1u);
              umma_bf16<2>(tmem_d, da_h, db_h, idesc, 1u);
            }
            umma_commit_pair_mask(empty_bar(stage), CL == 4 ? (uint16_t)15 : (uint16_t)3);
            if (++stage == STAGES) {
              stage = 0;
              phase ^= 1u;
            }
          }
          umma_commit_pair_mask(tfull_bar(acc), pair_mask);
          if (++acc == 2) {
            acc = 0;
            acc_phase ^= 1u;
          }
        }
      }
#ifdef TNN_F16_PROBE
      if (group == 0 || group == 37)
        printf("probe group %d: loop %lld cycles, wait full %lld, wait tmem-empty %lld\n", group,
               clock64() - t_begin, w_full, w_empty);
#endif
    }
  } else if (warp < EPI_WARP0) {
    if constexpr (NUM_THREADS == 384) asm volatile("setmaxnreg.dec.sync.aligned.u32 40;");
  } else {
    if constexpr (NUM_THREADS == 384) asm volatile("setmaxnreg.inc.sync.aligned.u32 216;");
    const int quad = warp & 3;
    const int half = (warp - EPI_WARP0) >> 2;
    int acc = 0;
    uint32_t acc_phase = 0;
    const bool relu = flags & 2;
    const int ec = -(meta_a->exp + meta_b->exp);
    const float f1 = pow2f(ec / 2), f2 = pow2f(ec - ec / 2);
    unsigned int st_max = 0u;
#ifdef TNN_F16_PROBE
    long long ep_wait = 0, ep_store = 0;
    const long long ep_begin = clock64();
#endif
    for (int u = group; u < num_units; u += num_groups) {
      int t, sp, kb_begin, kb_end;
      decode(u, t, sp, kb_begin, kb_end);
      const bool accumulate = (flags & 1) || sp > 0;
      const bool final_unit = (u < t_full || sp + 1 == tail_split);
      const bool emit_act = act_out != nullptr && final_unit;
      const bool want_stats = stat_out != nullptr && final_unit;
      const float* bias_u = sp == 0 ? bias : nullptr;
      int tm, tn;
      tile_coords((flags & 32) ? num_tiles - 1 - t : t, tiles_m, tiles_ns, group_m, tm, tn);
      if constexpr (CL == 4) tn = 2 * tn + (int)pair;
      const bool tile_valid = tn < tiles_n;
      const int flag_idx = tm * tiles_n + tn;
      const int col0 = tn * UMMA_N + half * 128;
      float sum[128];
#pragma unroll
      for (int j = 0; j < 128; ++j) sum[j] = 0.f;
      for (int kb0 = kb_begin; kb0 < kb_end; kb0 += CHUNK_KB) {
#ifdef TNN_F16_PROBE
        const long long q0 = clock64();
#endif
        mbar_wait(tfull_bar(acc), acc_phase);
#ifdef TNN_F16_PROBE
        ep_wait += clock64() - q0;
#endif
        tc_fence_after();
        const uint32_t taddr = tmem_base + ((uint32_t)(quad * 32) << 16) +
                               (uint32_t)(acc * UMMA_N + half * 128);
#pragma unroll
        for (int c = 0; c < 4; ++c) {
          uint32_t r[32];
          tmem_ld_32x32b_x32(taddr + (uint32_t)(c * 32), r);
          tmem_ld_wait();
#pragma unroll
          for (int j = 0; j < 32; ++j) sum[c * 32 + j] += __uint_as_float(r[j]);
        }
        tc_fence_before();
        __syncwarp();
        if (lane == 0) mbar_arrive_cluster_relaxed(tempty_bar(acc), 2 * pair);
        if (++acc == 2) {
          acc = 0;
          acc_phase ^= 1u;
        }
      }
      if (sp > 0 && tile_valid) {
        if (lane == 0) {
          const unsigned int need = (unsigned int)(sp * 16);
          unsigned int seen;
          long long t0 = clock64();
          do {
            asm volatile("ld.acquire.gpu.global.u32 %0, [%1];" : "=r"(seen) : "l"(tile_flags + flag_idx) : "memory");
            if (clock64() - t0 > 8000000000LL) {
              printf("tnn gemm_f16: split-K ordering wait timed out (tile %d split %d)\n", t, sp);
              __trap();
            }
          } while (seen < need);
        }
        __syncwarp();
        __threadfence();
      }
#ifdef TNN_F16_PROBE
      const long long q1 = clock64();
#endif
      {
        const int row_base = tm * TILE_M + (int)cta_rank * ROWS + quad * 32;
        float4* patch = reinterpret_cast<float4*>(smem_gen + STAGES * STAGE_BYTES + 256) + (warp - EPI_WARP0) * 256;
        const bool rows_aligned = (ldd % 4 == 0) && ((reinterpret_cast<uintptr_t>(D) & 15) == 0);
        const bool act_aligned = !emit_act || (((reinterpret_cast<uintptr_t>(act_out) |
                                                  reinterpret_cast<uintptr_t>(mask_src)) & 15) == 0);
        const bool want_mask = emit_act && mask_src != nullptr;
        const bool want_relu_side = !want_mask && (emit_act || (flags & 8));
        const float* pre_src = accumulate ? D : (want_mask ? mask_src : nullptr);
        const int rr = lane >> 3, c4l = lane & 7;
#pragma unroll 1
        for (int cb = 0; cb < 4; ++cb) {
          const int colb = col0 + cb * 32;
          if (colb >= N) break;
          switch (cb) {
            case 0: patch_write<0>(sum, patch, lane, f1, f2, bias_u, colb, N); break;
            case 1: patch_write<1>(sum, patch, lane, f1, f2, bias_u, colb, N); break;
            case 2: patch_write<2>(sum, patch, lane, f1, f2, bias_u, colb, N); break;
            default: patch_write<3>(sum, patch, lane, f1, f2, bias_u, colb, N); break;
          }
          __syncwarp();
          const int gcol = colb + c4l * 4;
          if (rows_aligned && act_aligned && colb + 32 <= N) {
            if (pre_src == nullptr) {
              const int nrows = min(32, M - row_base);
              const float4* pp0 = patch + rr * 8 + (c4l ^ rr);
              const float4* pp1 = patch + (rr + 4) * 8 + (c4l ^ (rr + 4));
              float* dp = D + (int64_t)(row_base + rr) * ldd + gcol;
              float* ap = emit_act ? act_out + (int64_t)(row_base + rr) * ldd + gcol : nullptr;
              const int64_t step = 4 * ldd;
#pragma unroll
              for (int i = 0; i < 8; ++i) {
                if (4 * i + rr < nrows) {
                  float4 v = (i & 1) ? pp1[(i >> 1) * 64] : pp0[(i >> 1) * 64];
                  if (relu) {
                    v.x = fmaxf(v.x, 0.f); v.y = fmaxf(v.y, 0.f);
                    v.z = fmaxf(v.z, 0.f); v.w = fmaxf(v.w, 0.f);
                  }
                  *reinterpret_cast<float4*>(dp) = v;
                  if (want_relu_side) {
                    v.x = v.x < 0.f ? 0.f : v.x; v.y = v.y < 0.f ? 0.f : v.y;
                    v.z = v.z < 0.f ? 0.f : v.z; v.w = v.w < 0.f ? 0.f : v.w;
                    if (emit_act) *reinterpret_cast<float4*>(ap) = v;
                  }
                  if (want_stats)
                    st_max = max(max(st_max, __float_as_uint(v.x) & 0x7FFFFFFFu),
                                 max(max(__float_as_uint(v.y) & 0x7FFFFFFFu, __float_as_uint(v.z) & 0x7FFFFFFFu),
                                     __float_as_uint(v.w) & 0x7FFFFFFFu));
                }
                dp += step;
                if (emit_act) ap += step;
              }
            } else {
              const int nrows = min(32, M - row_base);
              const float4* pp0 = patch + rr * 8 + (c4l ^ rr);
              const float4* pp1 = patch + (rr + 4) * 8 + (c4l ^ (rr + 4));
              const int64_t off0 = (int64_t)(row_base + rr) * ldd + gcol, step = 4 * ldd;
              float4 pre[8];
              {
                const float* sp_ = pre_src + off0;
#pragma unroll
                for (int i = 0; i < 8; ++i) {
                  if (4 * i + rr < nrows) pre[i] = *reinterpret_cast<const float4*>(sp_);
                  sp_ += step;
                }
              }
              float* dp = D + off0;
              float* ap = emit_act ? act_out + off0 : nullptr;
              const float* mp = (want_mask && accumulate) ? mask_src + off0 : nullptr;
#pragma unroll
              for (int i = 0; i < 8; ++i) {
                if (4 * i + rr < nrows) {
                  float4 v = (i & 1) ? pp1[(i >> 1) * 64] : pp0[(i >> 1) * 64];
                  if (accumulate) {
                    v.x += pre[i].x; v.y += pre[i].y; v.z += pre[i].z; v.w += pre[i].w;
                  }
                  if (relu) {
                    v.x = fmaxf(v.x, 0.f); v.y = fmaxf(v.y, 0.f);
                    v.z = fmaxf(v.z, 0.f); v.w = fmaxf(v.w, 0.f);
                  }
                  *reinterpret_cast<float4*>(dp) = v;
                  if (want_mask) {
                    const float4 z = accumulate ? *reinterpret_cast<const float4*>(mp) : pre[i];
                    v.x = z.x >= 0.f ? v.x : v.x * 0.f; v.y = z.y >= 0.f ? v.y : v.y * 0.f;
                    v.z = z.z >= 0.f ? v.z : v.z * 0.f; v.w = z.w >= 0.f ? v.w : v.w * 0.f;
                  } else if (want_relu_side) {
                    v.x = v.x < 0.f ? 0.f : v.x; v.y = v.y < 0.f ? 0.f : v.y;
                    v.z = v.z < 0.f ? 0.f : v.z; v.w = v.w < 0.f ? 0.f : v.w;
                  }
                  if (emit_act) *reinterpret_cast<float4*>(ap) = v;
                  if (want_stats)
                    st_max = max(max(st_max, __float_as_uint(v.x) & 0x7FFFFFFFu),
                                 max(max(__float_as_uint(v.y) & 0x7FFFFFFFu, __float_as_uint(v.z) & 0x7FFFFFFFu),
                                     __float_as_uint(v.w) & 0x7FFFFFFFu));
                }
                dp += step;
                if (emit_act) ap += step;
                if (mp) mp += step;
              }
            }
          } else {
#pragma unroll 1
            for (int i = 0; i < 8; ++i) {
              const int r = 4 * i + rr, grow = row_base + r;
              if (grow >= M) break;
              const float4 v4 = patch[r * 8 + (c4l ^ (r & 7))];
              const float s[4] = {v4.x, v4.y, v4.z, v4.w};
#pragma unroll 1
              for (int k = 0; k < 4; ++k) {
                if (gcol + k >= N) break;
                const int64_t off = (int64_t)grow * ldd + gcol + k;
                float x = k == 0 ? s[0] : (k == 1 ? s[1] : (k == 2 ? s[2] : s[3]));
                if (accumulate) x += D[off];
                if (relu) x = fmaxf(x, 0.f);
                D[off] = x;
                float a = x;
                if (want_mask) a = mask_src[off] >= 0.f ? x : x * 0.f;
                else if (want_relu_side) a = x < 0.f ? 0.f : x;
                if (emit_act) act_out[off] = a;
                if (want_stats) st_max = max(st_max, __float_as_uint(a) & 0x7FFFFFFFu);
              }
            }
          }
          __syncwarp();
        }
      }
#ifdef TNN_F16_PROBE
      ep_store += clock64() - q1;
#endif
      if (u >= t_full && sp + 1 < tail_split && tile_valid) {
        __threadfence();
        __syncwarp();
        if (lane == 0) atomicAdd(tile_flags + flag_idx, 1u);
      }
    }
#ifdef TNN_F16_PROBE
    if ((group == 0 || group == 37) && warp == 4 && lane == 0 && cta_rank == 0)
      printf("probe group %d epilogue warp 4: total %lld cycles, waiting for a chunk %lld, storing tiles %lld\n",
             group, clock64() - ep_begin, ep_wait, ep_store);
#endif
    if (stat_out != nullptr) {
      st_max = __reduce_max_sync(0xFFFFFFFFu, st_max);
      if (lane == 0 && st_max) atomicMax(&stat_out->absmax, st_max);
    }
  }

  __syncwarp();
  tc_fence_before();
  cluster_sync_all();
  if (warp == 1) {
    tc_fence_after();
    tmem_dealloc<2>(tmem_base, TMEM_COLS);
  }
}


__global__ void __launch_bounds__(256)
stats_kernel(const float* __restrict__ x, int64_t n, Meta* __restrict__ meta, int relu_mode, int vec,
             int only_if_needed) {
  if (only_if_needed && !meta->need_stats) return;
  unsigned int mx = 0u;
  const int64_t stride = (int64_t)gridDim.x * blockDim.x;
  auto take = [&](float v) {
    if (relu_mode && v < 0.f) v = 0.f;
    mx = max(mx, __float_as_uint(v) & 0x7FFFFFFFu);
  };
  if (vec) {
    const int64_t n4 = n / 4;
    const float4* x4 = reinterpret_cast<const float4*>(x);
    for (int64_t i = (int64_t)blockIdx.x * blockDim.x + threadIdx.x; i < n4; i += stride) {
      const float4 t = x4[i];
      take(t.x); take(t.y); take(t.z); take(t.w);
    }
    for (int64_t i = n4 * 4 + (int64_t)blockIdx.x * blockDim.x + threadIdx.x; i < n; i += stride) take(x[i]);
  } else {
    for (int64_t i = (int64_t)blockIdx.x * blockDim.x + threadIdx.x; i < n; i += stride) take(x[i]);
  }
  mx = __reduce_max_sync(0xFFFFFFFFu, mx);
  __shared__ unsigned int s_mx[8];
  const int warp = threadIdx.x >> 5, lane = threadIdx.x & 31;
  if (lane == 0) s_mx[warp] = mx;
  __syncthreads();
  if (threadIdx.x == 0) {
#pragma unroll
    for (int w = 1; w < 8; ++w) mx = max(mx, s_mx[w]);
    if (mx) atomicMax(&meta->absmax, mx);
  }
}

__global__ void __launch_bounds__(256)
split_f16_kernel(const float* __restrict__ x, int64_t R, int64_t C, __half* __restrict__ hf,
                 __half* __restrict__ l16, int64_t ld, Meta* __restrict__ meta, int relu_mode,
                 int vec_in) {
  int e, ok;
  meta_scale(meta->absmax, e, ok);
  const float sc = ok ? pow2f(e) : 1.f;
  const int64_t gpr = ld / 8;
  const int64_t total = R * gpr;
  const int64_t stride = (int64_t)gridDim.x * blockDim.x;
  unsigned int n_small = 0u, n_nz = 0u;
  if (ok) {
    for (int64_t i = (int64_t)blockIdx.x * blockDim.x + threadIdx.x; i < total; i += stride) {
      const int64_t r = i / gpr, c = (i - r * gpr) * 8;
      float v[8];
      if (vec_in && c + 7 < C) {
        const float4 t0 = *reinterpret_cast<const float4*>(x + r * C + c);
        const float4 t1 = *reinterpret_cast<const float4*>(x + r * C + c + 4);
        v[0] = t0.x; v[1] = t0.y; v[2] = t0.z; v[3] = t0.w;
        v[4] = t1.x; v[5] = t1.y; v[6] = t1.z; v[7] = t1.w;
      } else {
#pragma unroll
        for (int k = 0; k < 8; ++k) v[k] = (c + k < C) ? x[r * C + c + k] : 0.f;
      }
      union { __half2 h[4]; uint4 u; } ph, pl;
#pragma unroll
      for (int k = 0; k < 4; ++k) {
        float a = v[2 * k], b = v[2 * k + 1];
        if (relu_mode) { a = a < 0.f ? 0.f : a; b = b < 0.f ? 0.f : b; }
        a *= sc; b *= sc;
        n_nz += (a != 0.f) + (b != 0.f);
        n_small += (a != 0.f && fabsf(a) < SMALL_LIMIT) + (b != 0.f && fabsf(b) < SMALL_LIMIT);
        const __half2 h = __floats2half2_rn(a, b);
        const float2 hb = __half22float2(h);
        ph.h[k] = h;
        pl.h[k] = __floats2half2_rn(a - hb.x, b - hb.y);
      }
      *reinterpret_cast<uint4*>(hf + r * ld + c) = ph.u;
      *reinterpret_cast<uint4*>(l16 + r * ld + c) = pl.u;
    }
  }
  n_small = __reduce_add_sync(0xFFFFFFFFu, n_small);
  n_nz = __reduce_add_sync(0xFFFFFFFFu, n_nz);
  __shared__ unsigned int s_small[8], s_nz[8];
  const int warp = threadIdx.x >> 5, lane = threadIdx.x & 31;
  if (lane == 0) { s_small[warp] = n_small; s_nz[warp] = n_nz; }
  __syncthreads();
  if (threadIdx.x == 0) {
#pragma unroll
    for (int w = 1; w < 8; ++w) { n_small += s_small[w]; n_nz += s_nz[w]; }
    if (n_small) atomicAdd(&meta->n_small, n_small);
    if (n_nz) atomicAdd(&meta->n_nz, n_nz);
    __threadfence();
    if (atomicAdd(&meta->ticket, 1u) == gridDim.x - 1) {
      __threadfence();
      const unsigned int ts = *reinterpret_cast<volatile unsigned int*>(&meta->n_small);
      const unsigned int tn = *reinterpret_cast<volatile unsigned int*>(&meta->n_nz);
      meta->exp = e;
      meta->safe = (ok && (unsigned long long)ts * GUARD_FRACTION <= (unsigned long long)tn) ? 1 : 0;
    }
  }
}

static PFN_cuTensorMapEncodeTiled_v12000 g_encode = nullptr;

static int get_encode_fn() {
  if (g_encode) return 0;
  void* fn = nullptr;
  cudaDriverEntryPointQueryResult qres;
  TNN_CUDA(cudaGetDriverEntryPointByVersion("cuTensorMapEncodeTiled", &fn, 12000, cudaEnableDefault, &qres));
  if (qres != cudaDriverEntryPointSuccess || !fn) TNN_FAIL("cuTensorMapEncodeTiled is not available");
  g_encode = (PFN_cuTensorMapEncodeTiled_v12000)fn;
  return 0;
}

static int make_map(CUtensorMap* map, const void* ptr, int64_t rows, int64_t K, int64_t ld,
                    bool mn_major, int box_rows = ROWS) {
  if ((reinterpret_cast<uintptr_t>(ptr) & 15) != 0) TNN_FAIL("f16 GEMM: operand plane must be 16-byte aligned");
  if (ld % 8 != 0) TNN_FAIL("f16 GEMM: operand pitch must be a multiple of 8 elements");
  cuuint64_t dims[2] = {(cuuint64_t)(mn_major ? rows : K), (cuuint64_t)(mn_major ? K : rows)};
  cuuint64_t strides[1] = {(cuuint64_t)ld * 2};
  cuuint32_t box[2] = {(cuuint32_t)(mn_major ? 64 : BK), (cuuint32_t)(mn_major ? BK : box_rows)};
  cuuint32_t estr[2] = {1, 1};
  CUresult r = g_encode(map, CU_TENSOR_MAP_DATA_TYPE_FLOAT16, 2,
                        (void*)ptr, dims, strides, box, estr, CU_TENSOR_MAP_INTERLEAVE_NONE,
                        (mn_major || BK == 64) ? CU_TENSOR_MAP_SWIZZLE_128B : CU_TENSOR_MAP_SWIZZLE_64B,
                        CU_TENSOR_MAP_L2_PROMOTION_L2_256B,
                        CU_TENSOR_MAP_FLOAT_OOB_FILL_NONE);
  if (r != CUDA_SUCCESS) TNN_FAIL("cuTensorMapEncodeTiled (f16 planes) failed with code " + std::to_string((int)r));
  return 0;
}

static unsigned int* g_tile_flags = nullptr;
constexpr int MAX_FLAG_TILES = 1 << 16;
static bool g_attr_set[2][2][2] = {};
static int g_group_m = -8;
static bool g_reverse = true;
static int g_cluster = 2;

template <bool A_MN, bool B_MN, int CL>
static int launch(float* D, int64_t ldd, const void* a_h, const void* a_l, int64_t lda, const void* b_h,
                  const void* b_l, int64_t ldb, int64_t M, int64_t N, int64_t K, const float* bias,
                  int flags, float* act_out, const float* mask_src, const Meta* meta_a,
                  const Meta* meta_b, Meta* stat_out) {
  CUtensorMap ma_h, ma_l, mb_h, mb_l;
  if (make_map(&ma_h, a_h, M, K, lda, A_MN, CL == 4 ? 64 : KBOX_ROWS)) return 1;
  if (make_map(&ma_l, a_l, M, K, lda, A_MN, CL == 4 ? 64 : KBOX_ROWS)) return 1;
  if (make_map(&mb_h, b_h, N, K, ldb, B_MN, KBOX_ROWS)) return 1;
  if (make_map(&mb_l, b_l, N, K, ldb, B_MN, KBOX_ROWS)) return 1;
  auto kern = gemm_f16x3_kernel<A_MN, B_MN, CL>;
  if (!g_attr_set[A_MN][B_MN][CL == 4]) {
    TNN_CUDA(cudaFuncSetAttribute(kern, cudaFuncAttributeMaxDynamicSharedMemorySize, SMEM_BYTES));
    g_attr_set[A_MN][B_MN][CL == 4] = true;
  }
  const int64_t tiles_m = ceil_div(M, TILE_M), tiles_n = ceil_div(N, UMMA_N);
  const int64_t tiles = tiles_m * (CL == 4 ? ceil_div(tiles_n, 2) : tiles_n);
  const int max_groups = std::max(1, (ctx().sm_count - tc::g_reserved_sms) / CL);
  int t_full = (int)tiles, tail_split = 1;
  if (!(flags & 2) && tiles_m * tiles_n <= MAX_FLAG_TILES) {
    const int64_t num_kb = ceil_div(K, BK);
    const int64_t rem = tiles % max_groups;
    if (rem > 0) {
      int s = 1;
      while (s < 4 && rem * (s * 2) <= max_groups && num_kb / (s * 2) >= 512 / BK) s *= 2;
      if (s > 1) {
        t_full = (int)(tiles - rem);
        tail_split = s;
      }
    }
  }
  if (tail_split > 1) {
    if (!g_tile_flags) TNN_CUDA(cudaMalloc(&g_tile_flags, MAX_FLAG_TILES * sizeof(unsigned int)));
    TNN_CUDA(cudaMemsetAsync(g_tile_flags, 0, (size_t)(tiles_m * tiles_n) * sizeof(unsigned int), ctx().stream));
  }
  const int64_t units = t_full + (tiles - t_full) * tail_split;
  const int groups = (int)std::min<int64_t>(units, max_groups);
  cudaLaunchConfig_t cfg = {};
  cfg.gridDim = dim3((unsigned)(groups * CL));
  cfg.blockDim = dim3(NUM_THREADS);
  cfg.dynamicSmemBytes = SMEM_BYTES;
  cfg.stream = ctx().stream;
  cudaLaunchAttribute attr[1];
  attr[0].id = cudaLaunchAttributeClusterDimension;
  attr[0].val.clusterDim.x = CL;
  attr[0].val.clusterDim.y = 1;
  attr[0].val.clusterDim.z = 1;
  cfg.attrs = attr;
  cfg.numAttrs = 1;
  if constexpr (CL == 4) {
    static int max_clusters = 0;
    if (!max_clusters) {
      TNN_CUDA(cudaOccupancyMaxActiveClusters(&max_clusters, kern, &cfg));
      if (max_clusters < 1) max_clusters = 1;
    }
    if (groups > max_clusters) cfg.gridDim = dim3((unsigned)(max_clusters * CL));
  }
  const int gm = (CL == 4 && g_group_m < 0) ? std::min(-1, g_group_m / 2) : g_group_m;
  prof_begin(1);
  TNN_CUDA(cudaLaunchKernelEx(&cfg, kern, ma_h, ma_l, mb_h, mb_l, D, ldd, (int)M, (int)N, (int)K, bias, flags,
                              t_full, tail_split, g_tile_flags, act_out, mask_src, meta_a, meta_b, stat_out, gm));
  ctx().launches++;
  prof_end(1);
  return 0;
}

template <int CL>
static int launch_layout(int layout, float* D, int64_t ldd, const void* a_h, const void* a_l, int64_t lda,
                         const void* b_h, const void* b_l, int64_t ldb, int64_t M, int64_t N, int64_t K,
                         const float* bias, int flags, float* act_out, const float* mask_src,
                         const Meta* ma, const Meta* mb, Meta* st) {
  switch (layout & 3) {
    case 0: return launch<false, false, CL>(D, ldd, a_h, a_l, lda, b_h, b_l, ldb, M, N, K, bias, flags, act_out, mask_src, ma, mb, st);
    case 1: return launch<true, false, CL>(D, ldd, a_h, a_l, lda, b_h, b_l, ldb, M, N, K, bias, flags, act_out, mask_src, ma, mb, st);
    case 2: return launch<false, true, CL>(D, ldd, a_h, a_l, lda, b_h, b_l, ldb, M, N, K, bias, flags, act_out, mask_src, ma, mb, st);
    default: return launch<true, true, CL>(D, ldd, a_h, a_l, lda, b_h, b_l, ldb, M, N, K, bias, flags, act_out, mask_src, ma, mb, st);
  }
}

}
}

using namespace tnn;

extern "C" {

int tnn_set_gemm_f16_cluster(int cl) {
  if (cl != 2 && cl != 4) TNN_FAIL("tnn_set_gemm_f16_cluster: 2 (CTA pairs) or 4 (two pairs sharing A by TMA multicast)");
  f16::g_cluster = cl;
  return 0;
}

int tnn_f16_stats(const float* x, int64_t n, void* meta, int relu_mode) {
  TNN_REQUIRE_INIT();
  if (!meta) TNN_FAIL("tnn_f16_stats: meta is required");
  TNN_CUDA(cudaMemsetAsync(meta, 0, sizeof(f16::Meta), ctx().stream));
  if (n <= 0) return 0;
  const int vec = (reinterpret_cast<uintptr_t>(x) & 15) == 0;
  prof_begin(3);
  f16::stats_kernel<<<ew_grid(ceil_div(n, 16), 256), 256, 0, ctx().stream>>>(x, n, (f16::Meta*)meta, relu_mode, vec, 0);
  TNN_POST_LAUNCH();
  prof_end(3);
  return 0;
}

int tnn_f16_stats_cond(const float* x, int64_t n, void* meta, int relu_mode) {
  TNN_REQUIRE_INIT();
  if (!meta) TNN_FAIL("tnn_f16_stats_cond: meta is required");
  if (n <= 0) return 0;
  const int vec = (reinterpret_cast<uintptr_t>(x) & 15) == 0;
  prof_begin(3);
  f16::stats_kernel<<<ew_grid(ceil_div(n, 16), 256, 4), 256, 0, ctx().stream>>>(x, n, (f16::Meta*)meta, relu_mode, vec, 1);
  TNN_POST_LAUNCH();
  prof_end(3);
  return 0;
}

int tnn_f16_meta_reset(void* meta) {
  TNN_REQUIRE_INIT();
  if (!meta) TNN_FAIL("tnn_f16_meta_reset: meta is required");
  TNN_CUDA(cudaMemsetAsync(meta, 0, sizeof(f16::Meta), ctx().stream));
  return 0;
}

int tnn_split_f16(const float* x, int64_t R, int64_t C, void* hf, void* l16, int64_t ld, void* meta,
                  int relu_mode) {
  TNN_REQUIRE_INIT();
  if (R <= 0 || C <= 0) return 0;
  if (!hf || !l16 || !meta) TNN_FAIL("tnn_split_f16: both planes and the meta record are required");
  if (ld % 8 != 0 || ld < C) TNN_FAIL("tnn_split_f16: ld must be >= C and a multiple of 8");
  const int vec_in = (C % 4 == 0) && ((reinterpret_cast<uintptr_t>(x) & 15) == 0);
  prof_begin(3);
  f16::split_f16_kernel<<<ew_grid(R * (ld / 8), 256), 256, 0, ctx().stream>>>(
      x, R, C, (__half*)hf, (__half*)l16, ld, (f16::Meta*)meta, relu_mode, vec_in);
  TNN_POST_LAUNCH();
  prof_end(3);
  return 0;
}

int tnn_gemm_f16x3(float* D, int64_t ldd, const void* a_hf, const void* a_l16, int64_t lda,
                   const void* a_meta, const void* b_hf, const void* b_l16, int64_t ldb,
                   const void* b_meta, int64_t M, int64_t N, int64_t K, const float* bias, int flags,
                   int layout, float* act_out, const float* mask_src, void* stat_meta) {
  TNN_REQUIRE_INIT();
  if (M <= 0 || N <= 0) return 0;
  if (K <= 0) TNN_FAIL("tnn_gemm_f16x3: K must be positive");
  if (M > 2147483647LL || N > 2147483647LL || K > 2147483647LL) TNN_FAIL("tnn_gemm_f16x3: extent above int32");
  if (!a_meta || !b_meta) TNN_FAIL("tnn_gemm_f16x3: operand meta records are required");
  if (mask_src && !act_out) TNN_FAIL("tnn_gemm_f16x3: the mask_src form needs act_out");
  if (act_out && (flags & 2)) TNN_FAIL("tnn_gemm_f16x3: act_out and the relu-in-place flag are exclusive");
  if (f16::get_encode_fn()) return 1;
  if (getenv("TNN_EXP_FLAGS")) flags |= atoi(getenv("TNN_EXP_FLAGS")) & (128 | 256);
  static bool env_read = false;
  if (!env_read) {
    const char* gm = getenv("TNN_F16_GROUP_M");
    if (gm && atoi(gm) != 0 && atoi(gm) >= -64 && atoi(gm) <= 64) f16::g_group_m = atoi(gm);
    const char* rv = getenv("TNN_F16_REVERSE");
    if (rv) f16::g_reverse = atoi(rv) != 0;
    const char* cl = getenv("TNN_F16_CLUSTER");
    if (cl && (atoi(cl) == 2 || atoi(cl) == 4)) f16::g_cluster = atoi(cl);
    env_read = true;
  }
  if (f16::g_reverse) flags |= 32;
  const f16::Meta* ma = (const f16::Meta*)a_meta;
  const f16::Meta* mb = (const f16::Meta*)b_meta;
  f16::Meta* st = (f16::Meta*)stat_meta;
  if (f16::g_cluster == 4 && N > f16::UMMA_N)
    return f16::launch_layout<4>(layout, D, ldd, a_hf, a_l16, lda, b_hf, b_l16, ldb, M, N, K, bias, flags, act_out, mask_src, ma, mb, st);
  return f16::launch_layout<2>(layout, D, ldd, a_hf, a_l16, lda, b_hf, b_l16, ldb, M, N, K, bias, flags, act_out, mask_src, ma, mb, st);
}

}
```

Baseline: 1.063 million.

## Speculatively split f16 planes in one pass using per-site predicted scale exponents

Replaces the separate stats pass plus split pass with a one-pass kernel that splits using an exponent predicted from the previous step (stored in device-side prediction slots keyed by operand site), gathering absmax and counts at the same time. The follow-up split kernel validates the speculation: if the actual exponent matches, it only zeroes the padding and publishes meta, otherwise it redoes the full split. The CE backward kernel also writes the dz hi/lo planes directly using the predicted scale. This removes one full read pass over the activations per GEMM operand, at the cost of keeping a validation launch, a global prediction table, and a full re-split whenever the prediction misses.

```diff
diff --git a/core/_backend.py b/core/_backend.py
--- a/core/_backend.py
+++ b/core/_backend.py
@@ -95,10 +95,11 @@
     "tnn_gemm_tf32_bf16x2": [_c_vp, _c_i64, _c_vp, _c_vp, _c_vp, _c_i64, _c_vp, _c_vp, _c_vp, _c_i64,
                              _c_i64, _c_i64, _c_i64, _c_vp, _c_int, _c_int, _c_vp, _c_vp, _c_vp, _c_vp,
                              _c_i64, _c_vp],
-    "tnn_f16_stats": [_c_vp, _c_i64, _c_vp, _c_int],
+    "tnn_split_f16_onepass": [_c_vp, _c_i64, _c_i64, _c_vp, _c_vp, _c_i64, _c_vp, _c_int, _c_int],
+    "tnn_f16_full_splits": [_c_vp],
     "tnn_set_gemm_f16_cluster": [_c_int],
     "tnn_f16_meta_reset": [_c_vp],
-    "tnn_split_f16": [_c_vp, _c_i64, _c_i64, _c_vp, _c_vp, _c_i64, _c_vp, _c_int],
+    "tnn_split_f16": [_c_vp, _c_i64, _c_i64, _c_vp, _c_vp, _c_i64, _c_vp, _c_int, _c_int],
     "tnn_gemm_f16x3": [_c_vp, _c_i64, _c_vp, _c_vp, _c_i64, _c_vp, _c_vp, _c_vp, _c_i64, _c_vp, _c_i64,
                        _c_i64, _c_i64, _c_vp, _c_int, _c_int, _c_vp, _c_vp, _c_vp],
     "tnn_split_tf32_bf16_cond": [_c_vp, _c_i64, _c_i64, _c_vp, _c_vp, _c_vp, _c_i64, _c_int,
@@ -117,7 +118,7 @@
     "tnn_ce_loss": [_c_int, _c_vp, _c_int, _c_vp, _c_i64, _c_i64, _c_vp, _c_dbl, _c_vp, _c_vp, _c_vp],
     "tnn_ce_fwd_small": [_c_int, _c_vp, _c_int, _c_vp, _c_i64, _c_i64, _c_dbl, _c_vp, _c_vp, _c_vp, _c_vp],
     "tnn_ce_bwd": [_c_int, _c_vp, _c_vp, _c_int, _c_vp, _c_i64, _c_i64, _c_vp, _c_vp, _c_dbl, _c_vp, _c_vp,
-                   _c_vp],
+                   _c_vp, _c_vp, _c_vp, _c_i64, _c_int],
     "tnn_set_gemm_reserved_sms": [_c_int],
     "tnn_d2h_async": [_c_vp, _c_vp, _c_sz, _c_vp],
     "tnn_event_sync": [_c_vp],
@@ -780,10 +781,42 @@
 
 
 def _new_meta():
-    return empty((8,), F32)
-
-
-def split_planes_f16(x):
+    return empty((12,), F32)
+
+
+def _f16_ld(C):
+    return _round8(C) + F16_PITCH_PAD
+
+
+PRED_SLOTS = 4096
+_PRED_SLOT = {}
+
+
+def _pred_slot(key):
+    s = _PRED_SLOT.get(key)
+    if s is None:
+        if len(_PRED_SLOT) >= PRED_SLOTS:
+            _PRED_SLOT.clear()
+        s = _PRED_SLOT[key] = len(_PRED_SLOT)
+    return s
+
+
+def f16_full_splits():
+    n = _c_i64(0)
+    if _lib.tnn_f16_full_splits(ctypes.byref(n)):
+        _raise("tnn_f16_full_splits")
+    return n.value
+
+
+def _result_planes(cache, R, C, key):
+    ld = _f16_ld(C)
+    hf, l16 = _empty_16bit(R, ld), _empty_16bit(R, ld)
+    cache["planes"] = (hf, l16, ld)
+    cache["slot"] = _pred_slot(key)
+    return hf, l16, ld, cache["slot"]
+
+
+def split_planes_f16(x, key=None):
     cache = x.split
     if cache is None or cache.get("epoch") != _split_epoch:
         cache = {"epoch": _split_epoch}
@@ -791,7 +824,7 @@
     if "f" in cache:
         return cache["f"]
     R, C = x.shape
-    ld = _round8(C) + F16_PITCH_PAD
+    ld = _f16_ld(C)
     if type(x) is LazyReLU and x._real is None:
         src, relu_mode = x._src, 1
     else:
@@ -799,12 +832,20 @@
     meta = cache.get("stat")
     if meta is None:
         meta = _new_meta()
-        if _lib.tnn_f16_stats(src.ptr, R * C, meta.ptr, relu_mode):
-            _raise("tnn_f16_stats")
-    elif _lib.tnn_f16_stats_cond(src.ptr, R * C, meta.ptr, relu_mode):
-        _raise("tnn_f16_stats_cond")
-    hf, l16 = _empty_16bit(R, ld), _empty_16bit(R, ld)
-    if _lib.tnn_split_f16(src.ptr, R, C, hf.ptr, l16.ptr, ld, meta.ptr, relu_mode):
+        hf, l16 = _empty_16bit(R, ld), _empty_16bit(R, ld)
+        slot = _pred_slot(key) if key is not None else -1
+        if _lib.tnn_split_f16_onepass(src.ptr, R, C, hf.ptr, l16.ptr, ld, meta.ptr, relu_mode, slot):
+            _raise("tnn_split_f16_onepass")
+    else:
+        if _lib.tnn_f16_stats_cond(src.ptr, R * C, meta.ptr, relu_mode):
+            _raise("tnn_f16_stats_cond")
+        if "planes" in cache:
+            hf, l16, ld = cache["planes"]
+            slot = cache["slot"]
+        else:
+            hf, l16 = _empty_16bit(R, ld), _empty_16bit(R, ld)
+            slot = -1
+    if _lib.tnn_split_f16(src.ptr, R, C, hf.ptr, l16.ptr, ld, meta.ptr, relu_mode, slot):
         _raise("tnn_split_f16")
     cache["f"] = (hf, l16, ld, meta, src if src is not x else None, relu_mode)
     return cache["f"]
@@ -833,8 +874,8 @@
 
 
 def _matmul_f16(a, b, ta, tb, bias, out, flags, act, mask_src, M, N, K):
-    a_hf, a_l16, lda, a_meta, a_src, a_relu = split_planes_f16(a)
-    b_hf, b_l16, ldb, b_meta, b_src, b_relu = split_planes_f16(b)
+    a_hf, a_l16, lda, a_meta, a_src, a_relu = split_planes_f16(a, ("in", b.ptr, a.shape, ta, tb))
+    b_hf, b_l16, ldb, b_meta, b_src, b_relu = split_planes_f16(b, ("w", b.ptr, b.shape))
     a_src = a if a_src is None else a_src
     b_src = b if b_src is None else b_src
     layout = (1 if ta else 0) | (0 if tb else 2)
@@ -1110,16 +1151,21 @@
     if g.dtype != z.dtype:
         g = astype(g, z.dtype)
     stat = None
+    planes = (None, None, 0, -1)
     if z.dtype == F32 and TC_SPLIT == "f16" and TC_ENABLED and B * C >= (1 << 16):
         stat = _new_meta()
         if _lib.tnn_f16_meta_reset(stat.ptr):
             _raise("tnn_f16_meta_reset")
+        dz_split = {"epoch": _split_epoch, "stat": stat}
+        planes = _result_planes(dz_split, B, C, ("ce", B, C))
     y_ptr, lab_ptr = _ce_labels(y)
     if _lib.tnn_ce_bwd(_DT_CODE[z.dtype], dz.ptr, z.ptr, _DT_CODE[y.dtype], y_ptr, B, C, stats.ptr,
-                       q.ptr, float(m_global), g.ptr, stat.ptr if stat is not None else None, lab_ptr):
+                       q.ptr, float(m_global), g.ptr, stat.ptr if stat is not None else None, lab_ptr,
+                       planes[0].ptr if stat is not None else None, planes[1].ptr if stat is not None else None,
+                       planes[2], planes[3]):
         _raise("tnn_ce_bwd")
     if stat is not None:
-        dz.split = {"epoch": _split_epoch, "stat": stat}
+        dz.split = dz_split
     return dz
 
 
diff --git a/include/tnn_b200.h b/include/tnn_b200.h
--- a/include/tnn_b200.h
+++ b/include/tnn_b200.h
@@ -143,11 +143,14 @@
                          int64_t M, int64_t N, int64_t K, const float* bias, int flags, int layout,
                          float* act_out, float* act_hi, void* act_h16, void* act_l16, int64_t ld_act,
                          const float* mask_src);
-int tnn_f16_stats(const float* x, int64_t n, void* meta, int relu_mode);
+#define TNN_F16_PRED_SLOTS 4096
+int tnn_split_f16_onepass(const float* x, int64_t R, int64_t C, void* hf, void* l16, int64_t ld, void* meta,
+                          int relu_mode, int pred_slot);
+int tnn_f16_full_splits(int64_t* count);
 int tnn_set_gemm_f16_cluster(int cl);
 int tnn_f16_meta_reset(void* meta);
 int tnn_split_f16(const float* x, int64_t R, int64_t C, void* hf, void* l16, int64_t ld, void* meta,
-                  int relu_mode);
+                  int relu_mode, int pred_slot);
 int tnn_gemm_f16x3(float* D, int64_t ldd, const void* a_hf, const void* a_l16, int64_t lda,
                    const void* a_meta, const void* b_hf, const void* b_l16, int64_t ldb,
                    const void* b_meta, int64_t M, int64_t N, int64_t K, const float* bias, int flags,
@@ -182,7 +185,9 @@
 int tnn_ce_bwd(int dtype, void* dz, const void* z, int y_dtype, const void* y, int64_t B, int64_t C,
                const void* stats_dev, const void* q_dev, double m_global, const void* g_dev,
                void* stat_meta ,
-               const int32_t* labels_dev);
+               const int32_t* labels_dev,
+               void* dz_hf, void* dz_l16, int64_t ld ,
+               int pred_slot);
 
 int tnn_mlp_tail_workspace(int n_layers, const int64_t* in_dims, const int64_t* out_dims, int64_t batch,
                            int64_t* smem_bytes, int64_t* n_ctas, int64_t* scratch_floats);
diff --git a/tinynn-autograd_b200/build.py b/tinynn-autograd_b200/build.py
--- a/tinynn-autograd_b200/build.py
+++ b/tinynn-autograd_b200/build.py
@@ -12,7 +12,7 @@
 
 SOURCES = ["runtime.cu", "elementwise.cu", "reduce.cu", "layout.cu", "gemm_simt.cu",
            "gemm_tc.cu", "gemm_f16.cu", "fused.cu", "mlp_fused.cu", "comm.cu"]
-HEADERS = [os.path.join(CSRC, "common.cuh"), os.path.join(CSRC, "math.cuh"), os.path.join(CSRC, "tc_ptx.cuh"),
+HEADERS = [os.path.join(CSRC, "common.cuh"), os.path.join(CSRC, "f16_planes.cuh"), os.path.join(CSRC, "math.cuh"), os.path.join(CSRC, "tc_ptx.cuh"),
            os.path.join(ROOT, "include", "tnn_b200.h")]
 
 NVCC_FLAGS = ["-gencode", "arch=compute_100a,code=sm_100a", "-O3", "-lineinfo", "-std=c++17",
diff --git a/tinynn-autograd_b200/csrc/f16_planes.cuh b/tinynn-autograd_b200/csrc/f16_planes.cuh
--- /dev/null
+++ b/tinynn-autograd_b200/csrc/f16_planes.cuh
@@ -0,0 +1,90 @@
+#pragma once
+#include <cuda_fp16.h>
+
+#include "common.cuh"
+
+namespace tnn {
+namespace f16 {
+
+constexpr float SMALL_LIMIT = 0.03125f;
+constexpr unsigned int GUARD_FRACTION = 256;
+constexpr int PRED_SLOTS = TNN_F16_PRED_SLOTS;
+
+struct Meta {
+  unsigned int absmax;
+  unsigned int need_stats;
+  int exp;
+  int safe;
+  unsigned int n_small;
+  unsigned int n_nz;
+  unsigned int ticket;
+  int spec;
+  int spec_exp;
+  unsigned int spec_small;
+  unsigned int spec_nz;
+  unsigned int pad;
+};
+
+struct Pred {
+  int exp;
+  int valid;
+};
+
+Pred* pred_ptr(int slot);
+
+__device__ __forceinline__ void meta_scale(unsigned int amax_bits, int& e, int& ok) {
+  e = 0;
+  ok = 1;
+  if (amax_bits == 0u) return;
+  if (amax_bits >= 0x7F800000u) { ok = 0; return; }
+  const int ex = (int)(amax_bits >> 23) - 127;
+  if (ex < -112) { ok = 0; return; }
+  e = 14 - ex;
+}
+
+__device__ __forceinline__ float pow2f(int e) {
+  return __int_as_float((e + 127) << 23);
+}
+
+__device__ __forceinline__ void split2(float a, float b, float sc, __half2& h, __half2& l,
+                                       unsigned int& n_nz, unsigned int& n_small) {
+  a = __fmul_rn(a, sc);
+  b = __fmul_rn(b, sc);
+  n_nz += (a != 0.f) + (b != 0.f);
+  n_small += (a != 0.f && fabsf(a) < SMALL_LIMIT) + (b != 0.f && fabsf(b) < SMALL_LIMIT);
+  h = __floats2half2_rn(a, b);
+  const float2 hb = __half22float2(h);
+  l = __floats2half2_rn(__fsub_rn(a, hb.x), __fsub_rn(b, hb.y));
+}
+
+__device__ __forceinline__ void split4_store(float4 v, float sc, __half* hf, __half* l,
+                                             unsigned int& n_nz, unsigned int& n_small) {
+  union { __half2 h[2]; uint2 u; } ph, pl;
+  split2(v.x, v.y, sc, ph.h[0], pl.h[0], n_nz, n_small);
+  split2(v.z, v.w, sc, ph.h[1], pl.h[1], n_nz, n_small);
+  *reinterpret_cast<uint2*>(hf) = ph.u;
+  *reinterpret_cast<uint2*>(l) = pl.u;
+}
+
+__device__ __forceinline__ void split1_store(float a, float sc, __half* hf, __half* l,
+                                             unsigned int& n_nz, unsigned int& n_small) {
+  __half2 h, r;
+  unsigned int nz = 0u, sm = 0u;
+  split2(a, 0.f, sc, h, r, nz, sm);
+  n_nz += nz;
+  n_small += sm;
+  *hf = __low2half(h);
+  *l = __low2half(r);
+}
+
+__device__ __forceinline__ void spec_counts_flush(Meta* meta, unsigned int n_nz, unsigned int n_small) {
+  n_nz = __reduce_add_sync(0xFFFFFFFFu, n_nz);
+  n_small = __reduce_add_sync(0xFFFFFFFFu, n_small);
+  if ((threadIdx.x & 31) == 0) {
+    if (n_nz) atomicAdd(&meta->spec_nz, n_nz);
+    if (n_small) atomicAdd(&meta->spec_small, n_small);
+  }
+}
+
+}
+}
diff --git a/tinynn-autograd_b200/csrc/fused.cu b/tinynn-autograd_b200/csrc/fused.cu
--- a/tinynn-autograd_b200/csrc/fused.cu
+++ b/tinynn-autograd_b200/csrc/fused.cu
@@ -1,6 +1,7 @@
 #include <algorithm>
 
 #include "common.cuh"
+#include "f16_planes.cuh"
 #include "math.cuh"
 
 namespace tnn {
@@ -380,12 +381,20 @@
 template <typename T, typename TY, bool VEC>
 __global__ void __launch_bounds__(256)
 ce_bwd_kernel(T* dz, const T* z, const TY* y, int64_t B, int64_t C, const T* stats, const T* q,
-              T m, const T* gptr, unsigned int* absmax_out, const int32_t* labels) {
+              T m, const T* gptr, f16::Meta* meta, const int32_t* labels, __half* hf, __half* l16,
+              int64_t ld, const f16::Pred* pred) {
   constexpr int W = VEC ? 4 : 1;
   pdl_sync();
   const T mx = stats[0], S = stats[1], g = gptr[0];
   const int64_t nslot = C / W;
   unsigned int amax = 0u;
+  const bool planes = hf != nullptr && pred->valid;
+  const float psc = planes ? f16::pow2f(pred->exp) : 1.f;
+  unsigned int p_nz = 0u, p_small = 0u;
+  if (planes && blockIdx.x == 0 && blockIdx.y == 0 && threadIdx.x == 0) {
+    meta->spec = 1;
+    meta->spec_exp = pred->exp;
+  }
   for (int64_t r = blockIdx.y; r < B; r += gridDim.y) {
     const T qm = q[r] * m;
     const T* zr = z + r * C;
@@ -422,13 +431,23 @@
       }
       if constexpr (VEC) *reinterpret_cast<float4*>(dr + c * 4) = make_float4(out[0], out[1], out[2], out[3]);
       else dr[c] = out[0];
+      if constexpr (sizeof(T) == 4) {
+        if (planes) {
+          if constexpr (VEC)
+            f16::split4_store(make_float4(out[0], out[1], out[2], out[3]), psc, hf + r * ld + c * 4,
+                              l16 + r * ld + c * 4, p_nz, p_small);
+          else
+            f16::split1_store(out[0], psc, hf + r * ld + c, l16 + r * ld + c, p_nz, p_small);
+        }
+      }
     }
   }
   if constexpr (sizeof(T) == 4) {
-    if (absmax_out != nullptr) {
+    if (meta != nullptr) {
       amax = __reduce_max_sync(0xFFFFFFFFu, amax);
-      if ((threadIdx.x & 31) == 0 && amax) atomicMax(absmax_out, amax);
-    }
+      if ((threadIdx.x & 31) == 0 && amax) atomicMax(&meta->absmax, amax);
+    }
+    if (planes) f16::spec_counts_flush(meta, p_nz, p_small);
   }
 }
 
@@ -637,7 +656,8 @@
 
 template <typename T, typename TY>
 static int ce_bwd_impl(T* dz, const T* z, const TY* y, int64_t B, int64_t C, const T* stats,
-                       const T* q, double m, const T* g, unsigned int* absmax_out, const int32_t* labels) {
+                       const T* q, double m, const T* g, f16::Meta* meta, const int32_t* labels,
+                       __half* hf, __half* l16, int64_t ld, const f16::Pred* pred) {
   cudaStream_t st = ctx().stream;
   const bool vec = sizeof(T) == 4 && (C % 4 == 0) && al16(dz) && al16(z) && (labels || al16(y));
   const int64_t nslot = vec ? C / 4 : C;
@@ -648,10 +668,10 @@
   if (vec) {
     if constexpr (sizeof(T) == 4)
       TNN_CUDA(launch_small(ce_bwd_kernel<T, TY, true>, dim3(gx, (unsigned)gy), dim3(256), st, pdl, 1u,
-                            dz, z, y, B, C, stats, q, (T)m, g, absmax_out, labels));
+                            dz, z, y, B, C, stats, q, (T)m, g, meta, labels, hf, l16, ld, pred));
   } else {
     TNN_CUDA(launch_small(ce_bwd_kernel<T, TY, false>, dim3(gx, (unsigned)gy), dim3(256), st, pdl, 1u,
-                          dz, z, y, B, C, stats, q, (T)m, g, absmax_out, labels));
+                          dz, z, y, B, C, stats, q, (T)m, g, meta, labels, hf, l16, ld, pred));
   }
   ctx().launches++;
   return 0;
@@ -737,21 +757,33 @@
 
 int tnn_ce_bwd(int dtype, void* dz, const void* z, int y_dtype, const void* y, int64_t B, int64_t C,
                const void* stats_dev, const void* q_dev, double m_global, const void* g_dev,
-               void* stat_meta, const int32_t* labels_dev) {
+               void* stat_meta, const int32_t* labels_dev, void* dz_hf, void* dz_l16, int64_t ld,
+               int pred_slot) {
   TNN_REQUIRE_INIT();
   if (B <= 0 || C <= 0) return 0;
   if (!y && !labels_dev) TNN_FAIL("tnn_ce_bwd: neither dense labels nor class indices");
   const int32_t* lab = labels_dev;
-  unsigned int* am = (unsigned int*)stat_meta;
+  f16::Meta* am = (f16::Meta*)stat_meta;
   if (am && dtype != TNN_F32) TNN_FAIL("tnn_ce_bwd: operand statistics are float32 only");
+  const f16::Pred* pred = nullptr;
+  __half* ph = (__half*)dz_hf;
+  __half* pl = (__half*)dz_l16;
+  if (ph || pl) {
+    if (!ph || !pl || !am) TNN_FAIL("tnn_ce_bwd: dz planes need both planes and stat_meta");
+    if (ld % 8 != 0 || ld < C || ((reinterpret_cast<uintptr_t>(ph) | reinterpret_cast<uintptr_t>(pl)) & 15))
+      TNN_FAIL("tnn_ce_bwd: dz planes need 16-byte alignment and a pitch >= C, multiple of 8");
+    if (pred_slot < 0 || pred_slot >= f16::PRED_SLOTS) TNN_FAIL("tnn_ce_bwd: prediction slot out of range");
+    pred = f16::pred_ptr(pred_slot);
+    if (!pred) TNN_FAIL("tnn_ce_bwd: prediction slots are not available");
+  }
   if (dtype == TNN_F32 && y_dtype == TNN_F32)
-    return ce_bwd_impl<float, float>((float*)dz, (const float*)z, (const float*)y, B, C, (const float*)stats_dev, (const float*)q_dev, m_global, (const float*)g_dev, am, lab);
+    return ce_bwd_impl<float, float>((float*)dz, (const float*)z, (const float*)y, B, C, (const float*)stats_dev, (const float*)q_dev, m_global, (const float*)g_dev, am, lab, ph, pl, ld, pred);
   if (dtype == TNN_F32 && y_dtype == TNN_F64)
-    return ce_bwd_impl<float, double>((float*)dz, (const float*)z, (const double*)y, B, C, (const float*)stats_dev, (const float*)q_dev, m_global, (const float*)g_dev, am, lab);
+    return ce_bwd_impl<float, double>((float*)dz, (const float*)z, (const double*)y, B, C, (const float*)stats_dev, (const float*)q_dev, m_global, (const float*)g_dev, am, lab, ph, pl, ld, pred);
   if (dtype == TNN_F64 && y_dtype == TNN_F64)
-    return ce_bwd_impl<double, double>((double*)dz, (const double*)z, (const double*)y, B, C, (const double*)stats_dev, (const double*)q_dev, m_global, (const double*)g_dev, am, lab);
+    return ce_bwd_impl<double, double>((double*)dz, (const double*)z, (const double*)y, B, C, (const double*)stats_dev, (const double*)q_dev, m_global, (const double*)g_dev, am, lab, ph, pl, ld, pred);
   if (dtype == TNN_F64 && y_dtype == TNN_F32)
-    return ce_bwd_impl<double, float>((double*)dz, (const double*)z, (const float*)y, B, C, (const double*)stats_dev, (const double*)q_dev, m_global, (const double*)g_dev, am, lab);
+    return ce_bwd_impl<double, float>((double*)dz, (const double*)z, (const float*)y, B, C, (const double*)stats_dev, (const double*)q_dev, m_global, (const double*)g_dev, am, lab, ph, pl, ld, pred);
   TNN_FAIL("tnn_ce_bwd: bad dtype");
 }
 
diff --git a/tinynn-autograd_b200/csrc/gemm_f16.cu b/tinynn-autograd_b200/csrc/gemm_f16.cu
--- a/tinynn-autograd_b200/csrc/gemm_f16.cu
+++ b/tinynn-autograd_b200/csrc/gemm_f16.cu
@@ -7,6 +7,7 @@
 #include <cstdlib>
 
 #include "common.cuh"
+#include "f16_planes.cuh"
 #include "tc_ptx.cuh"
 
 namespace tnn {
@@ -45,34 +46,6 @@
 #endif
 constexpr int KBOX_ROWS = TNN_F16_KBOX_ROWS;
 constexpr int MN_BOX_BYTES = 64 * BK * 2;
-constexpr float SMALL_LIMIT = 0.03125f;
-constexpr unsigned int GUARD_FRACTION = 256;
-
-struct Meta {
-  unsigned int absmax;
-  unsigned int need_stats;
-  int exp;
-  int safe;
-  unsigned int n_small;
-  unsigned int n_nz;
-  unsigned int ticket;
-  unsigned int pad;
-};
-
-__device__ __forceinline__ void meta_scale(unsigned int amax_bits, int& e, int& ok) {
-  e = 0;
-  ok = 1;
-  if (amax_bits == 0u) return;
-  if (amax_bits >= 0x7F800000u) { ok = 0; return; }
-  const int ex = (int)(amax_bits >> 23) - 127;
-  if (ex < -112) { ok = 0; return; }
-  e = 14 - ex;
-}
-
-__device__ __forceinline__ float pow2f(int e) {
-  return __int_as_float((e + 127) << 23);
-}
-
 template <bool MN>
 __device__ __forceinline__ uint64_t make_desc(uint32_t saddr) {
   uint64_t d = 0;
@@ -611,9 +584,8 @@
 
 
 __global__ void __launch_bounds__(256)
-stats_kernel(const float* __restrict__ x, int64_t n, Meta* __restrict__ meta, int relu_mode, int vec,
-             int only_if_needed) {
-  if (only_if_needed && !meta->need_stats) return;
+stats_kernel(const float* __restrict__ x, int64_t n, Meta* __restrict__ meta, int relu_mode, int vec) {
+  if (!meta->need_stats) return;
   unsigned int mx = 0u;
   const int64_t stride = (int64_t)gridDim.x * blockDim.x;
   auto take = [&](float v) {
@@ -643,19 +615,51 @@
   }
 }
 
+__device__ Pred g_pred[PRED_SLOTS];
+__device__ unsigned long long g_full_splits = 0ull;
+
+__device__ __forceinline__ int guard_safe(int ok, unsigned int n_small, unsigned int n_nz) {
+  return (ok && (unsigned long long)n_small * GUARD_FRACTION <= (unsigned long long)n_nz) ? 1 : 0;
+}
+
+template <bool ONE_PASS>
 __global__ void __launch_bounds__(256)
 split_f16_kernel(const float* __restrict__ x, int64_t R, int64_t C, __half* __restrict__ hf,
                  __half* __restrict__ l16, int64_t ld, Meta* __restrict__ meta, int relu_mode,
-                 int vec_in) {
+                 int vec_in, Pred* __restrict__ pred) {
   int e, ok;
-  meta_scale(meta->absmax, e, ok);
+  const int64_t stride = (int64_t)gridDim.x * blockDim.x;
+  const int64_t tid = (int64_t)blockIdx.x * blockDim.x + threadIdx.x;
+  if constexpr (ONE_PASS) {
+    ok = pred != nullptr && pred->valid;
+    e = ok ? pred->exp : 0;
+  } else {
+    meta_scale(meta->absmax, e, ok);
+    if (ok && meta->spec && meta->spec_exp == e) {
+      const int64_t padw = ld - C;
+      if (padw > 0) {
+        for (int64_t i = tid; i < R * padw; i += stride) {
+          const int64_t r = i / padw, c = C + (i - r * padw);
+          hf[r * ld + c] = __float2half_rn(0.f);
+          l16[r * ld + c] = __float2half_rn(0.f);
+        }
+      }
+      if (tid == 0) {
+        meta->exp = e;
+        meta->n_small = meta->spec_small;
+        meta->n_nz = meta->spec_nz;
+        meta->safe = guard_safe(ok, meta->spec_small, meta->spec_nz);
+        if (pred) { pred->exp = e; pred->valid = 1; }
+      }
+      return;
+    }
+  }
   const float sc = ok ? pow2f(e) : 1.f;
   const int64_t gpr = ld / 8;
   const int64_t total = R * gpr;
-  const int64_t stride = (int64_t)gridDim.x * blockDim.x;
-  unsigned int n_small = 0u, n_nz = 0u;
-  if (ok) {
-    for (int64_t i = (int64_t)blockIdx.x * blockDim.x + threadIdx.x; i < total; i += stride) {
+  unsigned int n_small = 0u, n_nz = 0u, mx = 0u;
+  if (ok || ONE_PASS) {
+    for (int64_t i = tid; i < total; i += stride) {
       const int64_t r = i / gpr, c = (i - r * gpr) * 8;
       float v[8];
       if (vec_in && c + 7 < C) {
@@ -667,32 +671,42 @@
 #pragma unroll
         for (int k = 0; k < 8; ++k) v[k] = (c + k < C) ? x[r * C + c + k] : 0.f;
       }
+      if (relu_mode) {
+#pragma unroll
+        for (int k = 0; k < 8; ++k) v[k] = v[k] < 0.f ? 0.f : v[k];
+      }
+      if constexpr (ONE_PASS) {
+#pragma unroll
+        for (int k = 0; k < 8; ++k) mx = max(mx, __float_as_uint(v[k]) & 0x7FFFFFFFu);
+        if (!ok) continue;
+      }
       union { __half2 h[4]; uint4 u; } ph, pl;
 #pragma unroll
-      for (int k = 0; k < 4; ++k) {
-        float a = v[2 * k], b = v[2 * k + 1];
-        if (relu_mode) { a = a < 0.f ? 0.f : a; b = b < 0.f ? 0.f : b; }
-        a *= sc; b *= sc;
-        n_nz += (a != 0.f) + (b != 0.f);
-        n_small += (a != 0.f && fabsf(a) < SMALL_LIMIT) + (b != 0.f && fabsf(b) < SMALL_LIMIT);
-        const __half2 h = __floats2half2_rn(a, b);
-        const float2 hb = __half22float2(h);
-        ph.h[k] = h;
-        pl.h[k] = __floats2half2_rn(a - hb.x, b - hb.y);
-      }
+      for (int k = 0; k < 4; ++k) split2(v[2 * k], v[2 * k + 1], sc, ph.h[k], pl.h[k], n_nz, n_small);
       *reinterpret_cast<uint4*>(hf + r * ld + c) = ph.u;
       *reinterpret_cast<uint4*>(l16 + r * ld + c) = pl.u;
     }
   }
   n_small = __reduce_add_sync(0xFFFFFFFFu, n_small);
   n_nz = __reduce_add_sync(0xFFFFFFFFu, n_nz);
-  __shared__ unsigned int s_small[8], s_nz[8];
+  __shared__ unsigned int s_small[8], s_nz[8], s_mx[8];
   const int warp = threadIdx.x >> 5, lane = threadIdx.x & 31;
-  if (lane == 0) { s_small[warp] = n_small; s_nz[warp] = n_nz; }
+  if constexpr (ONE_PASS) mx = __reduce_max_sync(0xFFFFFFFFu, mx);
+  if (lane == 0) { s_small[warp] = n_small; s_nz[warp] = n_nz; s_mx[warp] = mx; }
   __syncthreads();
   if (threadIdx.x == 0) {
 #pragma unroll
-    for (int w = 1; w < 8; ++w) { n_small += s_small[w]; n_nz += s_nz[w]; }
+    for (int w = 1; w < 8; ++w) { n_small += s_small[w]; n_nz += s_nz[w]; mx = max(mx, s_mx[w]); }
+    if constexpr (ONE_PASS) {
+      if (mx) atomicMax(&meta->absmax, mx);
+      if (n_small) atomicAdd(&meta->spec_small, n_small);
+      if (n_nz) atomicAdd(&meta->spec_nz, n_nz);
+      if (ok && blockIdx.x == 0) {
+        meta->spec = 1;
+        meta->spec_exp = e;
+      }
+      return;
+    }
     if (n_small) atomicAdd(&meta->n_small, n_small);
     if (n_nz) atomicAdd(&meta->n_nz, n_nz);
     __threadfence();
@@ -701,9 +715,18 @@
       const unsigned int ts = *reinterpret_cast<volatile unsigned int*>(&meta->n_small);
       const unsigned int tn = *reinterpret_cast<volatile unsigned int*>(&meta->n_nz);
       meta->exp = e;
-      meta->safe = (ok && (unsigned long long)ts * GUARD_FRACTION <= (unsigned long long)tn) ? 1 : 0;
-    }
-  }
+      meta->safe = guard_safe(ok, ts, tn);
+      if (pred) { pred->exp = e; pred->valid = ok; }
+      atomicAdd(&g_full_splits, 1ull);
+    }
+  }
+}
+
+Pred* pred_ptr(int slot) {
+  static Pred* base = nullptr;
+  if (slot < 0) return nullptr;
+  if (!base && cudaGetSymbolAddress((void**)&base, g_pred) != cudaSuccess) return nullptr;
+  return base + slot;
 }
 
 static PFN_cuTensorMapEncodeTiled_v12000 g_encode = nullptr;
@@ -834,14 +857,20 @@
   return 0;
 }
 
-int tnn_f16_stats(const float* x, int64_t n, void* meta, int relu_mode) {
+int tnn_split_f16_onepass(const float* x, int64_t R, int64_t C, void* hf, void* l16, int64_t ld, void* meta,
+                          int relu_mode, int pred_slot) {
   TNN_REQUIRE_INIT();
-  if (!meta) TNN_FAIL("tnn_f16_stats: meta is required");
+  if (!hf || !l16 || !meta) TNN_FAIL("tnn_split_f16_onepass: both planes and the meta record are required");
+  if (ld % 8 != 0 || ld < C) TNN_FAIL("tnn_split_f16_onepass: ld must be >= C and a multiple of 8");
+  if (pred_slot >= f16::PRED_SLOTS) TNN_FAIL("tnn_split_f16_onepass: prediction slot out of range");
+  f16::Pred* pred = f16::pred_ptr(pred_slot);
+  if (pred_slot >= 0 && !pred) TNN_FAIL("tnn_split_f16_onepass: prediction slots are not available");
   TNN_CUDA(cudaMemsetAsync(meta, 0, sizeof(f16::Meta), ctx().stream));
-  if (n <= 0) return 0;
-  const int vec = (reinterpret_cast<uintptr_t>(x) & 15) == 0;
+  if (R <= 0 || C <= 0) return 0;
+  const int vec_in = (C % 4 == 0) && ((reinterpret_cast<uintptr_t>(x) & 15) == 0);
   prof_begin(3);
-  f16::stats_kernel<<<ew_grid(ceil_div(n, 16), 256), 256, 0, ctx().stream>>>(x, n, (f16::Meta*)meta, relu_mode, vec, 0);
+  f16::split_f16_kernel<true><<<ew_grid(R * (ld / 8), 256), 256, 0, ctx().stream>>>(
+      x, R, C, (__half*)hf, (__half*)l16, ld, (f16::Meta*)meta, relu_mode, vec_in, pred);
   TNN_POST_LAUNCH();
   prof_end(3);
   return 0;
@@ -853,9 +882,19 @@
   if (n <= 0) return 0;
   const int vec = (reinterpret_cast<uintptr_t>(x) & 15) == 0;
   prof_begin(3);
-  f16::stats_kernel<<<ew_grid(ceil_div(n, 16), 256, 4), 256, 0, ctx().stream>>>(x, n, (f16::Meta*)meta, relu_mode, vec, 1);
+  f16::stats_kernel<<<ew_grid(ceil_div(n, 16), 256, 4), 256, 0, ctx().stream>>>(x, n, (f16::Meta*)meta, relu_mode, vec);
   TNN_POST_LAUNCH();
   prof_end(3);
+  return 0;
+}
+
+int tnn_f16_full_splits(int64_t* count) {
+  TNN_REQUIRE_INIT();
+  if (!count) TNN_FAIL("tnn_f16_full_splits: count is required");
+  TNN_CUDA(cudaStreamSynchronize(ctx().stream));
+  unsigned long long n = 0;
+  TNN_CUDA(cudaMemcpyFromSymbol(&n, f16::g_full_splits, sizeof(n)));
+  *count = (int64_t)n;
   return 0;
 }
 
@@ -867,15 +906,18 @@
 }
 
 int tnn_split_f16(const float* x, int64_t R, int64_t C, void* hf, void* l16, int64_t ld, void* meta,
-                  int relu_mode) {
+                  int relu_mode, int pred_slot) {
   TNN_REQUIRE_INIT();
   if (R <= 0 || C <= 0) return 0;
   if (!hf || !l16 || !meta) TNN_FAIL("tnn_split_f16: both planes and the meta record are required");
   if (ld % 8 != 0 || ld < C) TNN_FAIL("tnn_split_f16: ld must be >= C and a multiple of 8");
+  if (pred_slot >= f16::PRED_SLOTS) TNN_FAIL("tnn_split_f16: prediction slot out of range");
+  f16::Pred* pred = f16::pred_ptr(pred_slot);
+  if (pred_slot >= 0 && !pred) TNN_FAIL("tnn_split_f16: prediction slots are not available");
   const int vec_in = (C % 4 == 0) && ((reinterpret_cast<uintptr_t>(x) & 15) == 0);
   prof_begin(3);
-  f16::split_f16_kernel<<<ew_grid(R * (ld / 8), 256), 256, 0, ctx().stream>>>(
-      x, R, C, (__half*)hf, (__half*)l16, ld, (f16::Meta*)meta, relu_mode, vec_in);
+  f16::split_f16_kernel<false><<<ew_grid(R * (ld / 8), 256), 256, 0, ctx().stream>>>(
+      x, R, C, (__half*)hf, (__half*)l16, ld, (f16::Meta*)meta, relu_mode, vec_in, pred);
   TNN_POST_LAUNCH();
   prof_end(3);
   return 0;
```

Result: no change. 1.053 million (median of 6 runs) (-0.9%).
